# vmonardo/pnp-svrg

Hardware: AMD Instinct MI355X
Metric: PnP-SVRG inner-iters/sec, 256x256 CSMRI+DnCNN (higher is better)
Workload: dtype f32; 1 GPU; pnp_svrg (true SVRG direction, T2=10, mb=1000) on 256x256 CSMRI, 20% Bernoulli mask, DnCNN-17 prox (reference DnCNN_noise15 weights); batch_per_gpu=120, problems_total=120, parallelism=replicas x1 (no data-path collective)

## Files before the change

include/pnp_hip.h:

```cpp
#ifndef PNP_HIP_H
#define PNP_HIP_H
#include <stddef.h>
#include <stdint.h>

#ifdef __cplusplus
extern "C" {
#endif

enum { PNP_F32 = 0, PNP_F64 = 1 };
enum { PNP_OK = 0, PNP_ERR_ARG = 1, PNP_ERR_HIP = 2, PNP_ERR_UNSUPPORTED = 3 };

int pnp_version(void);
const char* pnp_last_error(void);

typedef struct pnp_csmri_plan pnp_csmri_plan;

int pnp_csmri_plan_create(pnp_csmri_plan** plan, int H, int W, int batch, int dtype);
int pnp_csmri_plan_destroy(pnp_csmri_plan* plan);

int pnp_csmri_sel_from_indices(pnp_csmri_plan* plan, const int32_t* idx, int n, uint8_t* selT, void* stream);
int pnp_csmri_pack_mask(pnp_csmri_plan* plan, const uint8_t* selT, uint32_t* bitsT, void* stream);

int pnp_csmri_draw_thresholds(pnp_csmri_plan* plan, const uint32_t* bitsT, int mb, uint64_t seed, uint32_t step0,
                              int nsteps, const uint32_t* step_dev, void* mbd, uint32_t* selbits, void* stream);
int pnp_csmri_sel_from_thresholds(pnp_csmri_plan* plan, const uint32_t* bitsT, const void* mbd, uint8_t* selT,
                                  void* stream);
int pnp_csmri_draw_minibatch(pnp_csmri_plan* plan, const uint32_t* bitsT, int mb, uint64_t seed, uint32_t step,
                             const uint32_t* step_dev, uint8_t* selT, void* stream);
int pnp_csmri_sel_from_dense(pnp_csmri_plan* plan, const uint8_t* sel, uint8_t* selT, void* stream);

int pnp_csmri_pack_y(pnp_csmri_plan* plan, const void* YT, const uint8_t* selT, void* yh, void* stream);

int pnp_csmri_grad(pnp_csmri_plan* plan, const void* a, const void* b, const uint8_t* selT,
                   const void* yh, double alpha, double beta, const void* c1,
                   double gamma, const void* c2, void* out, void* stream);

int pnp_csmri_grad_sel(pnp_csmri_plan* plan, const void* a, const void* b, const uint8_t* selT, const uint32_t* bitsT,
                       const void* yh, const void* YT, double alpha, const void* alpha_vec, double beta,
                       const void* c1, double gamma, const void* c2, void* out, void* stream);

int pnp_csmri_svrg_step(pnp_csmri_plan* plan, const void* a, const void* b, const uint32_t* bitsT, double alpha,
                        const void* alpha_vec, double beta, const void* c1, double gamma, const void* c2, void* out,
                        int denoise, double sigma_modifier, double fallback_sigma, const void* xrec, double* sse_out,
                        void* sigma_out, void* stream);

int pnp_csmri_svrg_outer_step(pnp_csmri_plan* plan, const void* z, const uint32_t* mask_bitsT, const void* yh,
                              const void* alpha_vec, double lr, void* w_out, void* mu_out, void* out, int denoise,
                              double sigma_modifier, double fallback_sigma, const void* xrec, double* sse_out,
                              void* sigma_out, void* stream);

int pnp_csmri_svrg_outer_iteration(pnp_csmri_plan* plan, void* z, void* w, void* mu, const uint32_t* mask_bitsT, const void* yh,
                                   const void* alpha_vec, const uint32_t* selbits, int T2, double lr, int mini_batch_size,
                                   double sigma_modifier, double fallback_sigma, const void* xrec, double* sse_log,
                                   int log_row0, int n_log, void* sigma_out, void* stream);

typedef struct pnp_deblur_plan pnp_deblur_plan;
int pnp_deblur_plan_create(pnp_deblur_plan** plan, int H, int W, int batch, int dtype, const void* Bk, int M,
                           const int32_t* g_idx, const void* g_w, const int32_t* a_rowptr,
                           const int32_t* a_col, const void* a_val);
int pnp_deblur_plan_destroy(pnp_deblur_plan* plan);
int pnp_deblur_grad(pnp_deblur_plan* plan, const void* z, const void* Y, const uint8_t* sel, double scale,
                    void* out, void* stream);
int pnp_deblur_grad_mb(pnp_deblur_plan* plan, const void* z, const void* Y, const void* mbd, double scale,
                       void* out, void* stream);
int pnp_deblur_forward(pnp_deblur_plan* plan, const void* x, void* out, void* stream);

size_t pnp_pr_workspace_elems(int M, int N);
int pnp_pr_grad(const void* A, const void* w, const void* y, const int32_t* rows, int nsel, int M, int N,
                int dtype, double scale, void* workspace, void* out, void* stream);
int pnp_pr_grad_batch(const void* A, const void* w, const void* y, const int32_t* rows, int nsel, int M, int N, int batch,
                      int dtype, double scale, void* workspace, void* out, void* stream);
int pnp_pr_spectral_apply(const void* A, const void* v, const void* y, int M, int N, int dtype, double scale,
                          void* workspace, void* out, void* stream);

int pnp_sigma_est(const void* z, int H, int W, int batch, int dtype, void* sigma_out, void* stream);

int pnp_prox_tv(const void* z_in, void* z_out, int H, int W, int batch, int dtype,
                const void* sigma_in, double sigma_modifier, double fallback_sigma,
                const void* xrec, double* sse_out, void* sigma_out, void* stream);

int pnp_nlm2d(const void* z_in, void* z_out, int H, int W, int batch, int dtype, int patch_size,
              int patch_distance, const void* sigma_in, double sigma_modifier, double fixed_h,
              const double* w0, double w0_sum, const void* xrec, double* sse_out, double* sse_workspace,
              void* stream);

int pnp_sse(const void* z, const void* xrec, int n_per_problem, int batch, int dtype, double* sse_out, void* stream);

int pnp_minmax(const void* z, int n_per_problem, int batch, int dtype, void* out, void* stream);

typedef struct pnp_dncnn_plan pnp_dncnn_plan;
int pnp_dncnn_plan_create(pnp_dncnn_plan** plan, int n_mid, const float* w_first, const float* w_mid,
                          const float* b_mid, const float* w_last, int H, int W, int batch);
int pnp_dncnn_plan_destroy(pnp_dncnn_plan* plan);
int pnp_dncnn_set_affine(pnp_dncnn_plan* plan, const float* b_first, float b_last, float negative_slope);
int pnp_dncnn_set_winograd(pnp_dncnn_plan* plan, int enable);
int pnp_dncnn_forward(pnp_dncnn_plan* plan, const float* x, float* r, void* stream);
int pnp_dncnn_denoise(pnp_dncnn_plan* plan, const void* z_in, void* z_out, int dtype, double sigma_net,
                      const void* xrec, double* sse_out, void* stream);

int pnp_mmo_denoise(pnp_dncnn_plan* plan, const void* z_in, void* z_out, int dtype, const void* xrec,
                    double* sse_out, void* stream);

int pnp_dncnn_profile_begin(pnp_dncnn_plan* plan, int max_calls);
int pnp_dncnn_profile_end(pnp_dncnn_plan* plan, double* avg_ms_per_launch, long* launches);
int pnp_dncnn_debug_clock(pnp_dncnn_plan* plan, int reps, double* cycles, double* ref_ticks, void* stream);
size_t pnp_dncnn_debug_w44_floats(void);
int pnp_dncnn_debug_w44_weights(pnp_dncnn_plan* plan, int layer, float* dst, void* stream);
int pnp_dncnn_debug_mid_layer(pnp_dncnn_plan* plan, int layer, const float* in, float* out, const float* w44_override,
                              int w44_rows, void* stream);
int pnp_dncnn_debug_fused_last(pnp_dncnn_plan* plan, const float* in, float* part, int w44_rows, void* stream);

int pnp_counter_add(uint32_t* counter, uint32_t inc, void* stream);
int pnp_log_append(const double* src, int n, double* log, int n_log, const uint32_t* step_dev, void* stream);
int pnp_log_append_inc(const double* src, int n, double* log, int n_log, uint32_t* counter, void* stream);

int pnp_draw_thresholds(int M, int batch, int mb, uint64_t seed, uint32_t step0, int nsteps, const uint32_t* step_dev,
                        void* mbd, void* stream);
int pnp_indicator_from_thresholds(int M, int batch, const void* mbd, uint8_t* sel, void* stream);
int pnp_rows_from_thresholds(int M, int batch, int mb, const void* mbd, int32_t* rows, void* stream);
int pnp_indicator_from_indices(const int32_t* idx, int n, int M, int batch, uint8_t* sel, void* stream);
int pnp_saga_table_update(void* z, const void* g, void* slot, const void* prev, void* sum, double lr, double inv_hist,
                          size_t n, int dtype, void* stream);

int pnp_axpbypcz(double a, const void* x, double b, const void* y, double c, const void* w,
                 void* out, size_t n, int dtype, void* stream);

int pnp_legacy_choice(uint32_t* mt_key, int* mt_pos, const int64_t* pool, int pop, int size, int32_t* work, int64_t* out);

#ifdef __cplusplus
}
#endif
#endif
```

pnp_svrg_amd/_native.py:

```python
import ctypes
import os

_HERE = os.path.dirname(os.path.abspath(__file__))
LIB_PATH = os.environ.get('PNP_HIP_LIB') or os.path.join(_HERE, 'lib', 'libpnp_hip.so')

F32, F64 = 0, 1

_vp = ctypes.c_void_p
_i = ctypes.c_int
_d = ctypes.c_double
_sz = ctypes.c_size_t

SIGNATURES = {
    'pnp_version': (_i, []),
    'pnp_last_error': (ctypes.c_char_p, []),
    'pnp_csmri_plan_create': (_i, [ctypes.POINTER(_vp), _i, _i, _i, _i]),
    'pnp_csmri_plan_destroy': (_i, [_vp]),
    'pnp_csmri_sel_from_indices': (_i, [_vp, _vp, _i, _vp, _vp]),
    'pnp_csmri_pack_mask': (_i, [_vp, _vp, _vp, _vp]),
    'pnp_csmri_draw_thresholds': (_i, [_vp, _vp, _i, ctypes.c_uint64, ctypes.c_uint32, _i, _vp, _vp, _vp, _vp]),
    'pnp_csmri_sel_from_thresholds': (_i, [_vp, _vp, _vp, _vp, _vp]),
    'pnp_csmri_draw_minibatch': (_i, [_vp, _vp, _i, ctypes.c_uint64, ctypes.c_uint32, _vp, _vp, _vp]),
    'pnp_counter_add': (_i, [_vp, ctypes.c_uint32, _vp]),
    'pnp_log_append': (_i, [_vp, _i, _vp, _i, _vp, _vp]),
    'pnp_log_append_inc': (_i, [_vp, _i, _vp, _i, _vp, _vp]),
    'pnp_csmri_sel_from_dense': (_i, [_vp, _vp, _vp, _vp]),
    'pnp_csmri_pack_y': (_i, [_vp, _vp, _vp, _vp, _vp]),
    'pnp_csmri_grad': (_i, [_vp, _vp, _vp, _vp, _vp, _d, _d, _vp, _d, _vp, _vp, _vp]),
    'pnp_csmri_grad_sel': (_i, [_vp, _vp, _vp, _vp, _vp, _vp, _vp, _d, _vp, _d, _vp, _d, _vp, _vp, _vp]),
    'pnp_csmri_svrg_step': (_i, [_vp, _vp, _vp, _vp, _d, _vp, _d, _vp, _d, _vp, _vp, _i, _d, _d, _vp, _vp, _vp, _vp]),
    'pnp_csmri_svrg_outer_step': (_i, [_vp, _vp, _vp, _vp, _vp, _d, _vp, _vp, _vp, _i, _d, _d, _vp, _vp, _vp, _vp]),
    'pnp_csmri_svrg_outer_iteration': (_i, [_vp, _vp, _vp, _vp, _vp, _vp, _vp, _vp, _i, _d, _i, _d, _d, _vp, _vp, _i, _i, _vp, _vp]),
    'pnp_deblur_plan_create': (_i, [ctypes.POINTER(_vp), _i, _i, _i, _i, _vp, _i, _vp, _vp, _vp, _vp, _vp]),
    'pnp_deblur_plan_destroy': (_i, [_vp]),
    'pnp_deblur_grad': (_i, [_vp, _vp, _vp, _vp, _d, _vp, _vp]),
    'pnp_deblur_grad_mb': (_i, [_vp, _vp, _vp, _vp, _d, _vp, _vp]),
    'pnp_deblur_forward': (_i, [_vp, _vp, _vp, _vp]),
    'pnp_pr_workspace_elems': (_sz, [_i, _i]),
    'pnp_pr_grad': (_i, [_vp, _vp, _vp, _vp, _i, _i, _i, _i, _d, _vp, _vp, _vp]),
    'pnp_pr_grad_batch': (_i, [_vp, _vp, _vp, _vp, _i, _i, _i, _i, _i, _d, _vp, _vp, _vp]),
    'pnp_pr_spectral_apply': (_i, [_vp, _vp, _vp, _i, _i, _i, _d, _vp, _vp, _vp]),
    'pnp_sigma_est': (_i, [_vp, _i, _i, _i, _i, _vp, _vp]),
    'pnp_prox_tv': (_i, [_vp, _vp, _i, _i, _i, _i, _vp, _d, _d, _vp, _vp, _vp, _vp]),
    'pnp_nlm2d': (_i, [_vp, _vp, _i, _i, _i, _i, _i, _i, _vp, _d, _d, _vp, _d, _vp, _vp, _vp, _vp]),
    'pnp_sse': (_i, [_vp, _vp, _i, _i, _i, _vp, _vp]),
    'pnp_minmax': (_i, [_vp, _i, _i, _i, _vp, _vp]),
    'pnp_dncnn_plan_create': (_i, [ctypes.POINTER(_vp), _i, _vp, _vp, _vp, _vp, _i, _i, _i]),
    'pnp_dncnn_plan_destroy': (_i, [_vp]),
    'pnp_dncnn_set_affine': (_i, [_vp, _vp, ctypes.c_float, ctypes.c_float]),
    'pnp_dncnn_set_winograd': (_i, [_vp, _i]),
    'pnp_dncnn_forward': (_i, [_vp, _vp, _vp, _vp]),
    'pnp_dncnn_denoise': (_i, [_vp, _vp, _vp, _i, _d, _vp, _vp, _vp]),
    'pnp_mmo_denoise': (_i, [_vp, _vp, _vp, _i, _vp, _vp, _vp]),
    'pnp_dncnn_profile_begin': (_i, [_vp, _i]),
    'pnp_dncnn_profile_end': (_i, [_vp, ctypes.POINTER(_d), ctypes.POINTER(ctypes.c_long)]),
    'pnp_dncnn_debug_clock': (_i, [_vp, _i, ctypes.POINTER(_d), ctypes.POINTER(_d), _vp]),
    'pnp_dncnn_debug_w44_floats': (_sz, []),
    'pnp_dncnn_debug_w44_weights': (_i, [_vp, _i, _vp, _vp]),
    'pnp_dncnn_debug_mid_layer': (_i, [_vp, _i, _vp, _vp, _vp, _i, _vp]),
    'pnp_dncnn_debug_fused_last': (_i, [_vp, _vp, _vp, _i, _vp]),
    'pnp_draw_thresholds': (_i, [_i, _i, _i, ctypes.c_uint64, ctypes.c_uint32, _i, _vp, _vp, _vp]),
    'pnp_indicator_from_thresholds': (_i, [_i, _i, _vp, _vp, _vp]),
    'pnp_rows_from_thresholds': (_i, [_i, _i, _i, _vp, _vp, _vp]),
    'pnp_indicator_from_indices': (_i, [_vp, _i, _i, _i, _vp, _vp]),
    'pnp_saga_table_update': (_i, [_vp, _vp, _vp, _vp, _vp, _d, _d, _sz, _i, _vp]),
    'pnp_axpbypcz': (_i, [_d, _vp, _d, _vp, _d, _vp, _vp, _sz, _i, _vp]),
    'pnp_legacy_choice': (_i, [_vp, ctypes.POINTER(ctypes.c_int), _vp, _i, _i, _vp, _vp]),
}

_lib = None


class NativeError(RuntimeError):
    pass


def lib():
    global _lib
    if _lib is None:
        if not os.path.exists(LIB_PATH):
            raise NativeError(
                f'{LIB_PATH} not found: build it with `python -c "import __graft_entry__ as g; g.build()"` '
                '(or `make -C pnp_svrg_amd/csrc`). There is no CPU fallback.')
        h = ctypes.CDLL(LIB_PATH)
        for name, (res, args) in SIGNATURES.items():
            fn = getattr(h, name)
            fn.restype = res
            fn.argtypes = args
        _lib = h
    return _lib


def check(status, what=''):
    if status != 0:
        msg = lib().pnp_last_error().decode(errors='replace')
        raise NativeError(f'{what} failed (status {status}): {msg}')


def call(name, *args):
    check(getattr(lib(), name)(*args), name)
```

pnp_svrg_amd/csrc/dncnn.hip:

```cpp
#include "direct.h"
#include "wino44.h"
#include "wino44b.h"
#include "reduce.h"
#include <vector>
#include <algorithm>
#include <cstdlib>
#include <type_traits>

namespace pnp {

constexpr int C = 64;

template <typename T>
__global__ __launch_bounds__(256) void k_first(const T* __restrict__ z, const T* __restrict__ mm,
                                               const float* __restrict__ w, const float* __restrict__ bfirst,
                                               float* __restrict__ out, int H, int W, double srange, double sshift,
                                               int clamp01, float slope) {
    __shared__ float ws[C * 9];
    __shared__ float bs[C];
    for (int i = threadIdx.x; i < C * 9; i += 256) ws[i] = w[i];
    if (threadIdx.x < C) bs[threadIdx.x] = bfirst[threadIdx.x];
    __syncthreads();
    const int b = blockIdx.y;
    const int p = blockIdx.x * 256 + threadIdx.x;
    if (p >= H * W) return;
    const int y = p / W, x = p - y * W;
    const T lo = mm ? mm[2 * b] : (T)0, hi = mm ? mm[2 * b + 1] : (T)1;
    const T* zi = z + (size_t)b * H * W;
    float v[9];
#pragma unroll
    for (int t = 0; t < 9; ++t) {
        const int yy = y + t / 3 - 1, xx = x + t % 3 - 1;
        float q = 0.f;
        if (yy >= 0 && yy < H && xx >= 0 && xx < W) {
            T u = zi[yy * W + xx];
            if (clamp01) {
                u = u < (T)0 ? (T)0 : (u > (T)1 ? (T)1 : u);
            } else {
                u = (u - lo) / (hi - lo);
                u = u * (T)srange + (T)sshift;
            }
            q = (float)u;
        }
        v[t] = q;
    }
#pragma unroll 4
    for (int c = 0; c < C; ++c) {
        float a = 0.f;
#pragma unroll
        for (int t = 0; t < 9; ++t) a = fmaf(ws[c * 9 + t], v[t], a);
        a += bs[c];
        out[((size_t)b * C + c) * H * W + p] = a > 0.f ? a : slope * a + 0.f;
    }
}

constexpr int LT_R = 16, LT_C = 64, LT_CK = 4, LT_PR = LT_R + 2, LT_PC = LT_C + 8;

template <typename T>
__global__ __launch_bounds__(256) void k_last(const float* __restrict__ act, const float* __restrict__ w,
                                              const T* zin, const T* __restrict__ mm,
                                              T* zout, float* __restrict__ r_out,
                                              const T* __restrict__ xrec, double* __restrict__ sse_part, int H, int W,
                                              double srange, double sshift, int skip01, float blast) {
    __shared__ float ws[C * 9];
    __shared__ __attribute__((aligned(16))) float tile[LT_CK * LT_PR * LT_PC];
    __shared__ double red[4];
    const int tid = threadIdx.x;
    for (int i = tid; i < C * 9; i += 256) ws[i] = w[i];
    const int b = blockIdx.z;
    const int ty0 = blockIdx.y * LT_R, tx0 = blockIdx.x * LT_C;
    const int py = tid >> 4, px = (tid & 15) * 4;
    const float* ab = act + (size_t)b * C * H * W;
    float r[4] = {0.f, 0.f, 0.f, 0.f};
    constexpr int SLAB = LT_CK * LT_PR * (LT_PC / 4);
    constexpr int PER_T = (SLAB + 255) / 256;
    float4 pre[PER_T];
    auto fetch = [&](int c0) {
#pragma unroll
        for (int k = 0; k < PER_T; ++k) {
            const int i = tid + 256 * k;
            float4 v = make_float4(0.f, 0.f, 0.f, 0.f);
            if (i < SLAB) {
                const int ch = i / (LT_PR * (LT_PC / 4)), rem = i - ch * (LT_PR * (LT_PC / 4));
                const int ry = rem / (LT_PC / 4), cx = rem - ry * (LT_PC / 4);
                const int y = ty0 - 1 + ry, x = tx0 - 4 + 4 * cx;
                if (y >= 0 && y < H && x >= 0 && x < W)
                    v = *reinterpret_cast<const float4*>(ab + ((size_t)(c0 + ch) * H + y) * W + x);
            }
            pre[k] = v;
        }
    };
    fetch(0);
    for (int c0 = 0; c0 < C; c0 += LT_CK) {
        __syncthreads();
#pragma unroll
        for (int k = 0; k < PER_T; ++k) {
            const int i = tid + 256 * k;
            if (i < SLAB) reinterpret_cast<float4*>(tile)[i] = pre[k];
        }
        __syncthreads();
        if (c0 + LT_CK < C) fetch(c0 + LT_CK);
#pragma unroll
        for (int ch = 0; ch < LT_CK; ++ch) {
            const float* wc = ws + (c0 + ch) * 9;
#pragma unroll
            for (int dy = 0; dy < 3; ++dy) {
                const float* row = tile + (ch * LT_PR + py + dy) * LT_PC + px + 4;
                const float4 m = *reinterpret_cast<const float4*>(row);
                const float l = row[-1], rr = row[4];
                const float w0 = wc[dy * 3], w1 = wc[dy * 3 + 1], w2 = wc[dy * 3 + 2];
                r[0] = fmaf(w0, l, fmaf(w1, m.x, fmaf(w2, m.y, r[0])));
                r[1] = fmaf(w0, m.x, fmaf(w1, m.y, fmaf(w2, m.z, r[1])));
                r[2] = fmaf(w0, m.y, fmaf(w1, m.z, fmaf(w2, m.w, r[2])));
                r[3] = fmaf(w0, m.z, fmaf(w1, m.w, fmaf(w2, rr, r[3])));
            }
        }
    }
    double err = 0.0;
    const int y = ty0 + py;
    if (y < H) {
#pragma unroll
        for (int j = 0; j < 4; ++j) {
            const int x = tx0 + px + j;
            if (x >= W) continue;
            const size_t p = (size_t)b * H * W + (size_t)y * W + x;
            r[j] += blast;
            if (r_out != nullptr) r_out[p] = r[j];
            if (zout != nullptr && skip01) {
                const float xin = (float)zin[p];
                float v = (xin < 0.f ? 0.f : (xin > 1.f ? 1.f : xin)) + r[j];
                v = v < 0.f ? 0.f : (v > 1.f ? 1.f : v);
                zout[p] = (T)v;
                if (xrec != nullptr) {
                    const double d = (double)xrec[p] - (double)(T)v;
                    err += d * d;
                }
            } else if (zout != nullptr) {
                const T lo = mm[2 * b], hi = mm[2 * b + 1];
                T v = (zin[p] - lo) / (hi - lo);
                v = v * (T)srange + (T)sshift;
                v = v - (T)r[j];
                v = (v - (T)sshift) / (T)srange;
                v = v * (hi - lo) + lo;
                zout[p] = v;
                if (xrec != nullptr) {
                    const double d = (double)xrec[p] - (double)v;
                    err += d * d;
                }
            }
        }
    }
    if (sse_part != nullptr) {
        err = wave_sum(err);
        if ((tid & 63) == 0) red[tid >> 6] = err;
        __syncthreads();
        if (tid == 0)
            sse_part[((size_t)b * gridDim.y + blockIdx.y) * gridDim.x + blockIdx.x] = red[0] + red[1] + red[2] + red[3];
    }
}

template <typename T>
__global__ __launch_bounds__(256) void k_last_patches(const float* __restrict__ part, const T* zin, const T* __restrict__ mm,
                                                      T* zout, float* __restrict__ r_out, const T* __restrict__ xrec,
                                                      double* __restrict__ sse_part, int H, int W, double srange, double sshift,
                                                      float blast) {
    __shared__ double red[4];
    const int tid = threadIdx.x, b = blockIdx.z;
    const int iy = tid >> 6, ix = tid & 3, bx = blockIdx.x * 16 + ((tid >> 2) & 15), by = blockIdx.y;
    const int y = 4 * by + iy, x = 4 * bx + ix;
    const int NBX = W / 4, NBY = H / 4;
    const float* pb = part + (size_t)b * NBY * NBX * 36;
    auto at = [&](int qy, int qx, int py, int px) { return pb[((size_t)qy * NBX + qx) * 36 + py * 6 + px]; };
    const int vy = iy == 0 ? -1 : iy == 3 ? 1 : 0, vx = ix == 0 ? -1 : ix == 3 ? 1 : 0;
    const bool hv = vy != 0 && by + vy >= 0 && by + vy < NBY, hh = vx != 0 && bx + vx >= 0 && bx + vx < NBX;
    const int py = iy + 1, px = ix + 1, pyn = py - 4 * vy, pxn = px - 4 * vx;
    float r = at(by, bx, py, px);
    if (hv) r += at(by + vy, bx, pyn, px);
    if (hh) r += at(by, bx + vx, py, pxn);
    if (hv && hh) r += at(by + vy, bx + vx, pyn, pxn);
    r += blast;
    const size_t p = (size_t)b * H * W + (size_t)y * W + x;
    if (r_out != nullptr) r_out[p] = r;
    double err = 0.0;
    if (zout != nullptr) {
        const T lo = mm ? mm[2 * b] : (T)0, hi = mm ? mm[2 * b + 1] : (T)1;
        T v = (zin[p] - lo) / (hi - lo);
        v = v * (T)srange + (T)sshift;
        v = v - (T)r;
        v = (v - (T)sshift) / (T)srange;
        v = v * (hi - lo) + lo;
        zout[p] = v;
        if (xrec != nullptr) {
            const double d = (double)xrec[p] - (double)v;
            err = d * d;
        }
    }
    if (sse_part != nullptr) {
        err = wave_sum(err);
        if ((tid & 63) == 0) red[tid >> 6] = err;
        __syncthreads();
        if (tid == 0)
            sse_part[((size_t)b * gridDim.y + blockIdx.y) * gridDim.x + blockIdx.x] = red[0] + red[1] + red[2] + red[3];
    }
}

__global__ void k_sum_parts(const double* __restrict__ part, int nparts, double* __restrict__ out) {
    double s = 0;
    for (int i = threadIdx.x; i < nparts; i += 64) s += part[(size_t)blockIdx.x * nparts + i];
    s = wave_sum(s);
    if (threadIdx.x == 0) out[blockIdx.x] = s;
}

}
using namespace pnp;

static const ConvMode kModes[] = {
    {0, direct_supports, direct_layer_bytes, direct_pack, direct_layer, direct_debug_clock, false},
    {1, direct_supports, wino23_layer_bytes, wino23_pack, wino23_layer, wino23_debug_clock, false},
    {5, wino44_supports, wino44_layer_bytes, wino44_pack, wino44_layer, wino44_debug_clock, true},
    {6, wino44b_supports, wino44b_layer_bytes, wino44b_pack, wino44b_layer, wino44b_debug_clock, false},
};
constexpr int NMODES = sizeof(kModes) / sizeof(kModes[0]);

static const ConvMode* find_mode(int mode) {
    for (const ConvMode& m : kModes)
        if (m.mode == mode) return &m;
    return nullptr;
}

static int resolve_conv_mode(int requested, int H, int W, bool strict, const ConvMode** out) {
    const ConvMode* m = find_mode(requested);
    PNP_CHECK_ARG(m || !strict,
                  "mode must be 0 (direct), 1 (Winograd F(2,3) along x), 5 (Winograd F(4x4,3x3)) or 6 (the same on 3 x bf16 splits)");
    if (!m) m = find_mode(5);
    PNP_CHECK_ARG(m->supports(H, W) || !strict, "Winograd F(4x4,3x3) needs H % 8 == 0 and W % 64 == 0");
    *out = m->supports(H, W) ? m : find_mode(1);
    return PNP_OK;
}

struct pnp_dncnn_plan {
    int n_mid, H, W, batch, num_cu;
    float *w_first, *w_last, *bias;
    void* wconv[NMODES];
    const ConvMode* conv;
    float* b_first;
    float b_last, slope;
    bool edge_fusion;
    float* part;
    float *act0, *act1, *zeros;
    double* mm;
    double* sse_part;
    bool profile;
    std::vector<hipEvent_t> ev;
    size_t ev_used;
    double prof_ms;
    long prof_launches;
};

static void plan_free(pnp_dncnn_plan* p) {
    for (void* q : p->wconv) (void)hipFree(q);
    for (void* q : {(void*)p->bias, (void*)p->w_first, (void*)p->w_last, (void*)p->act0, (void*)p->act1, (void*)p->zeros,
                    (void*)p->mm, (void*)p->sse_part, (void*)p->b_first, (void*)p->part})
        (void)hipFree(q);
    for (hipEvent_t e : p->ev) (void)hipEventDestroy(e);
    delete p;
}

static ConvLayerArgs conv_args(const pnp_dncnn_plan* p, int l, const float* in, float* out, hipStream_t s) {
    return {in, out, p->wconv[p->conv - kModes], l, p->bias + (size_t)l * C, p->zeros, p->H, p->W, p->batch, p->num_cu, p->slope, s};
}

extern "C" int pnp_dncnn_plan_create(pnp_dncnn_plan** out, int n_mid, const float* w_first, const float* w_mid,
                                     const float* b_mid, const float* w_last, int H, int W, int batch) {
    PNP_CHECK_ARG(out && w_first && w_mid && b_mid && w_last, "null argument");
    PNP_CHECK_ARG(n_mid >= 1 && batch >= 1, "n_mid and batch must be >= 1");
    PNP_CHECK_ARG(H % 8 == 0 && W % 32 == 0 && (H * W) % 256 == 0, "H must be a multiple of 8, W of 32");
    auto* p = new pnp_dncnn_plan{};
    p->n_mid = n_mid; p->H = H; p->W = W; p->batch = batch;
    hipDeviceProp_t prop;
    int dev = 0;
    PNP_CHECK_HIP(hipGetDevice(&dev));
    PNP_CHECK_HIP(hipGetDeviceProperties(&prop, dev));
    p->num_cu = prop.multiProcessorCount;
    const char* ev = getenv("PNP_DNCNN_WINOGRAD");
    (void)resolve_conv_mode(ev ? atoi(ev) : 5, H, W, false, &p->conv);
    const char* ef = getenv("PNP_DNCNN_EDGE_FUSION");
    p->edge_fusion = !(ef && atoi(ef) == 0);
    const size_t act_bytes = (size_t)batch * C * H * W * sizeof(float);
    hipError_t e = hipSuccess;
    auto alloc = [&](auto** dst, size_t bytes, const void* src = nullptr) {
        if (e == hipSuccess) e = hipMalloc(dst, bytes);
        if (e == hipSuccess && src) e = hipMemcpy(*dst, src, bytes, hipMemcpyHostToDevice);
    };
    for (int i = 0; i < NMODES; ++i) {
        if (!kModes[i].supports(H, W)) continue;
        std::vector<char> w(kModes[i].layer_bytes() * n_mid);
        kModes[i].pack(w_mid, n_mid, w.data());
        alloc(&p->wconv[i], w.size(), w.data());
    }
    alloc(&p->bias, (size_t)n_mid * C * sizeof(float), b_mid);
    alloc(&p->w_first, C * 9 * sizeof(float), w_first);
    alloc(&p->w_last, C * 9 * sizeof(float), w_last);
    alloc(&p->b_first, C * sizeof(float));
    if (e == hipSuccess) e = hipMemset(p->b_first, 0, C * sizeof(float));
    alloc(&p->act0, act_bytes);
    alloc(&p->act1, act_bytes);
    alloc(&p->zeros, 256);
    if (e == hipSuccess) e = hipMemset(p->zeros, 0, 256);
    alloc(&p->mm, (size_t)batch * 2 * sizeof(double));
    alloc(&p->sse_part, (size_t)batch * (H * W / 256) * sizeof(double));
    if (wino44_supports(H, W)) alloc(&p->part, wino44_part_floats(H, W, batch) * sizeof(float));
    if (e != hipSuccess) {
        set_error(std::string("pnp_dncnn_plan_create: ") + hipGetErrorString(e));
        plan_free(p);
        return PNP_ERR_HIP;
    }
    *out = p;
    return PNP_OK;
}

extern "C" int pnp_dncnn_plan_destroy(pnp_dncnn_plan* p) {
    if (p) plan_free(p);
    return PNP_OK;
}

namespace {
template <typename T>
int run_dncnn(pnp_dncnn_plan* p, const T* z_in, bool normalise, double sigma_net, T* z_out, float* r_out,
              const T* xrec, double* sse_out, hipStream_t s, bool mmo = false) {
    const int H = p->H, W = p->W, B = p->batch, HW = H * W;
    T* mm = normalise ? (T*)p->mm : nullptr;
    double srange = 1.0, sshift = 0.0;
    if (normalise) {
        k_minmax<T><<<B, 256, 0, s>>>(z_in, HW, mm);
        PNP_CHECK_LAUNCH();
        srange = 1.0 + sigma_net / 255.0 / 2.0;
        sshift = (1.0 - srange) / 2.0;
    }
    dim3 pg(HW / 256, B);
    k_first<T><<<pg, 256, 0, s>>>(z_in, mm, p->w_first, p->b_first, p->act0, H, W, srange, sshift, mmo ? 1 : 0, p->slope);
    PNP_CHECK_LAUNCH();
    float *src = p->act0, *dst = p->act1;
    const bool fuse_last = p->edge_fusion && p->conv->fuses_last && p->slope == 0.f && !mmo && std::is_same<T, float>::value &&
                           p->part != nullptr;
    const bool prof = p->profile && p->ev_used + 2 <= p->ev.size();
    if (prof) PNP_CHECK_HIP(hipEventRecord(p->ev[p->ev_used], s));
    for (int l = 0; l < p->n_mid; ++l) {
        ConvLayerArgs a = conv_args(p, l, src, dst, s);
        if (fuse_last && l == p->n_mid - 1) { a.wlast = p->w_last; a.part = p->part; }
        const int rc = p->conv->layer(a);
        if (rc != PNP_OK) return rc;
        std::swap(src, dst);
    }
    if (prof) { PNP_CHECK_HIP(hipEventRecord(p->ev[p->ev_used + 1], s)); p->ev_used += 2; }
    if (fuse_last) {
        const dim3 fg(W / 64, H / 4, B);
        k_last_patches<T><<<fg, 256, 0, s>>>(p->part, z_in, mm, z_out, r_out, xrec, sse_out ? p->sse_part : nullptr, H, W, srange,
                                             sshift, p->b_last);
        PNP_CHECK_LAUNCH();
        if (sse_out) {
            k_sum_parts<<<B, 64, 0, s>>>(p->sse_part, (int)(fg.x * fg.y), sse_out);
            PNP_CHECK_LAUNCH();
        }
        return PNP_OK;
    }
    dim3 lg((W + LT_C - 1) / LT_C, (H + LT_R - 1) / LT_R, B);
    k_last<T><<<lg, 256, 0, s>>>(src, p->w_last, z_in, mm, z_out, r_out, xrec, sse_out ? p->sse_part : nullptr, H, W,
                                 srange, sshift, mmo ? 1 : 0, p->b_last);
    PNP_CHECK_LAUNCH();
    if (sse_out) {
        k_sum_parts<<<B, 64, 0, s>>>(p->sse_part, (int)(lg.x * lg.y), sse_out);
        PNP_CHECK_LAUNCH();
    }
    return PNP_OK;
}
}

extern "C" size_t pnp_dncnn_debug_w44_floats(void) { return wino44_layer_bytes() / sizeof(float); }

extern "C" int pnp_dncnn_debug_w44_weights(pnp_dncnn_plan* p, int layer, float* dst, void* stream) {
    PNP_CHECK_ARG(p && dst && layer >= 0 && layer < p->n_mid, "bad argument");
    const char* w = (const char*)p->wconv[find_mode(5) - kModes];
    PNP_CHECK_ARG(w != nullptr, "the plan's image size rules out the F(4x4,3x3) kernel (mode 5): no such weights");
    PNP_CHECK_HIP(hipMemcpyAsync(dst, w + (size_t)layer * wino44_layer_bytes(), wino44_layer_bytes(), hipMemcpyDeviceToDevice,
                                 (hipStream_t)stream));
    return PNP_OK;
}

extern "C" int pnp_dncnn_debug_mid_layer(pnp_dncnn_plan* p, int layer, const float* in, float* out, const float* w44_override,
                                         int w44_rows, void* stream) {
    PNP_CHECK_ARG(p && in && out && layer >= 0 && layer < p->n_mid && w44_rows >= 0 && w44_rows <= 2, "bad argument");
    ConvLayerArgs a = conv_args(p, layer, in, out, (hipStream_t)stream);
    a.force_rows = w44_rows;
    a.w44_override = w44_override;
    return p->conv->layer(a);
}

extern "C" int pnp_dncnn_debug_fused_last(pnp_dncnn_plan* p, const float* in, float* part, int w44_rows, void* stream) {
    PNP_CHECK_ARG(p && in && part && w44_rows >= 0 && w44_rows <= 2, "bad argument");
    ConvLayerArgs a = conv_args(p, p->n_mid - 1, in, nullptr, (hipStream_t)stream);
    a.force_rows = w44_rows;
    a.wlast = p->w_last;
    a.part = part;
    return p->conv->layer(a);
}

extern "C" int pnp_dncnn_set_affine(pnp_dncnn_plan* p, const float* b_first, float b_last, float negative_slope) {
    PNP_CHECK_ARG(p != nullptr, "null plan");
    PNP_CHECK_ARG(negative_slope >= 0.f && negative_slope < 1.f, "negative_slope must be in [0, 1)");
    if (b_first) PNP_CHECK_HIP(hipMemcpy(p->b_first, b_first, C * sizeof(float), hipMemcpyHostToDevice));
    else PNP_CHECK_HIP(hipMemset(p->b_first, 0, C * sizeof(float)));
    p->b_last = b_last;
    p->slope = negative_slope;
    return PNP_OK;
}

extern "C" int pnp_dncnn_set_winograd(pnp_dncnn_plan* p, int enable) {
    PNP_CHECK_ARG(p != nullptr, "null plan");
    return resolve_conv_mode(enable, p->H, p->W, true, &p->conv);
}

extern "C" int pnp_dncnn_profile_begin(pnp_dncnn_plan* p, int max_calls) {
    PNP_CHECK_ARG(p && max_calls > 0, "bad argument");
    while (p->ev.size() < (size_t)2 * max_calls) {
        hipEvent_t e;
        PNP_CHECK_HIP(hipEventCreate(&e));
        p->ev.push_back(e);
    }
    p->profile = true; p->ev_used = 0; p->prof_ms = 0; p->prof_launches = 0;
    return PNP_OK;
}

extern "C" int pnp_dncnn_profile_end(pnp_dncnn_plan* p, double* avg_ms_per_launch, long* launches) {
    PNP_CHECK_ARG(p && avg_ms_per_launch && launches, "null argument");
    p->profile = false;
    for (size_t i = 0; i + 1 < p->ev_used; i += 2) {
        PNP_CHECK_HIP(hipEventSynchronize(p->ev[i + 1]));
        float ms = 0;
        PNP_CHECK_HIP(hipEventElapsedTime(&ms, p->ev[i], p->ev[i + 1]));
        p->prof_ms += ms;
        p->prof_launches += p->n_mid;
    }
    *launches = p->prof_launches;
    *avg_ms_per_launch = p->prof_launches ? p->prof_ms / (double)p->prof_launches : 0.0;
    return PNP_OK;
}

extern "C" int pnp_dncnn_debug_clock(pnp_dncnn_plan* p, int reps, double* cycles, double* ref_ticks, void* stream) {
    PNP_CHECK_ARG(p && cycles && ref_ticks && reps >= 1, "bad argument");
    std::vector<double> c, r;
    const int rc = p->conv->debug_clock(conv_args(p, 0, p->act0, p->act1, (hipStream_t)stream), reps, c, r);
    if (rc != PNP_OK) return rc;
    std::sort(c.begin(), c.end());
    std::sort(r.begin(), r.end());
    *cycles = c[c.size() / 2];
    *ref_ticks = r[r.size() / 2];
    return PNP_OK;
}

extern "C" int pnp_dncnn_forward(pnp_dncnn_plan* p, const float* x, float* r, void* stream) {
    PNP_CHECK_ARG(p && x && r, "null argument");
    return run_dncnn<float>(p, x, false, 0.0, nullptr, r, nullptr, nullptr, (hipStream_t)stream);
}

extern "C" int pnp_mmo_denoise(pnp_dncnn_plan* p, const void* z_in, void* z_out, int dtype, const void* xrec,
                               double* sse_out, void* stream) {
    PNP_CHECK_ARG(p && z_in && z_out, "null argument");
    PNP_CHECK_ARG(!(sse_out && !xrec), "sse_out needs xrec");
    if (dtype == PNP_F32)
        return run_dncnn<float>(p, (const float*)z_in, false, 0.0, (float*)z_out, nullptr, (const float*)xrec, sse_out,
                                (hipStream_t)stream, true);
    if (dtype == PNP_F64)
        return run_dncnn<double>(p, (const double*)z_in, false, 0.0, (double*)z_out, nullptr, (const double*)xrec, sse_out,
                                 (hipStream_t)stream, true);
    PNP_CHECK_ARG(false, "bad dtype");
}

extern "C" int pnp_dncnn_denoise(pnp_dncnn_plan* p, const void* z_in, void* z_out, int dtype, double sigma_net,
                                 const void* xrec, double* sse_out, void* stream) {
    PNP_CHECK_ARG(p && z_in && z_out, "null argument");
    PNP_CHECK_ARG(!(sse_out && !xrec), "sse_out needs xrec");
    if (dtype == PNP_F32)
        return run_dncnn<float>(p, (const float*)z_in, true, sigma_net, (float*)z_out, nullptr, (const float*)xrec, sse_out,
                                (hipStream_t)stream);
    if (dtype == PNP_F64)
        return run_dncnn<double>(p, (const double*)z_in, true, sigma_net, (double*)z_out, nullptr, (const double*)xrec,
                                 sse_out, (hipStream_t)stream);
    PNP_CHECK_ARG(false, "bad dtype");
}
```

pnp_svrg_amd/csrc/dncnn_conv.h:

```cpp
#pragma once
#include "common.h"
#include <vector>

namespace pnp {

struct ConvLayerArgs {
    const float* in;
    float* out;
    const void* w;
    int layer;
    const float *bias, *zeros;
    int H, W, batch, num_cu;
    float slope;
    hipStream_t s;
    int force_rows = 0;
    const float* w44_override = nullptr;
    const float* wlast = nullptr;
    float* part = nullptr;
};

struct ConvMode {
    int mode;
    bool (*supports)(int H, int W);
    size_t (*layer_bytes)();
    void (*pack)(const float* w_mid, int n_mid, void* out);
    int (*layer)(const ConvLayerArgs& a);
    int (*debug_clock)(const ConvLayerArgs& a, int reps, std::vector<double>& cycles, std::vector<double>& ticks);
    bool fuses_last;
};

inline int check_plain_conv(const ConvLayerArgs& a) {
    PNP_CHECK_ARG(a.w44_override == nullptr, "w44_override needs the F(4x4,3x3) kernel (mode 5)");
    PNP_CHECK_ARG(a.part == nullptr, "the fused last layer needs the F(4x4,3x3) kernel (mode 5) and ReLU");
    return PNP_OK;
}

template <typename F>
int read_stamps(hipStream_t s, int nwg, int per_wg, F&& launch, std::vector<unsigned long long>& h, std::vector<double>& cycles,
                std::vector<double>& ticks) {
    unsigned long long* d = nullptr;
    PNP_CHECK_HIP(hipMalloc(&d, (size_t)nwg * per_wg * sizeof(*d)));
    h.resize((size_t)nwg * per_wg);
    const int rc = launch(d);
    hipError_t e = rc != PNP_OK ? hipSuccess : hipMemcpyAsync(h.data(), d, h.size() * sizeof(*d), hipMemcpyDeviceToHost, s);
    if (rc == PNP_OK && e == hipSuccess) e = hipStreamSynchronize(s);
    (void)hipFree(d);
    if (rc != PNP_OK) return rc;
    PNP_CHECK_HIP(e);
    for (int i = 0; i < nwg; ++i) { cycles.push_back((double)h[(size_t)per_wg * i]); ticks.push_back((double)h[(size_t)per_wg * i + 1]); }
    return PNP_OK;
}

}
```

pnp_svrg_amd/csrc/dncnn_wino44.hip:

```cpp
#include "common.h"
#include "wino44.h"
#include "tilewalk.h"
#include <vector>
#include <utility>
#include <cstdlib>

namespace pnp {
namespace w44 {

using f32x4 = __attribute__((ext_vector_type(4))) float;
using f32x2 = __attribute__((ext_vector_type(2))) float;

constexpr int C = 64;
constexpr int TC = 64;
constexpr int PC = 72;
constexpr int KC = 8;
constexpr int NCH = C / KC;
template <int NG_> struct Geo {
    static constexpr int NG = NG_;
    static constexpr int TR = 4 * NG, PR = TR + 2;
    static constexpr int PLANE = NG == 2 ? 768 : 512;
    static constexpr int DBUF = KC * PLANE;
    static constexpr int PPW = DBUF / 256 / 4;
    static constexpr int VPL = 128 * NG;
    static constexpr int VBUF = 36 * VPL;
    static constexpr int LDS_FLOATS = 2 * DBUF + 2 * VBUF;
    static constexpr int NQ_AGPR = NG == 2 ? 64 : 36;
    static constexpr bool in_agpr(int g, int xi) { return g * 36 + xi < NQ_AGPR; }
};
constexpr int URING = 18;
constexpr unsigned DUMMY = 1u << 27;

__device__ __forceinline__ void bt6(float d0, float d1, float d2, float d3, float d4, float d5, float (&v)[6]) {
    const float t1 = __builtin_fmaf(-4.f, d2, d4), t2 = __builtin_fmaf(-4.f, d1, d3);
    const float t3 = d4 - d2, sd = d3 - d1;
    v[0] = __builtin_fmaf(4.f, d0, __builtin_fmaf(-5.f, d2, d4));
    v[1] = t1 + t2;
    v[2] = t1 - t2;
    v[3] = __builtin_fmaf(2.f, sd, t3);
    v[4] = __builtin_fmaf(-2.f, sd, t3);
    v[5] = __builtin_fmaf(4.f, d1, __builtin_fmaf(-5.f, d3, d5));
}
template <typename T> __device__ __forceinline__ void at6(T m0, T m1, T m2, T m3, T m4, T m5, T (&y)[4]) {
    const T s12 = m1 + m2, d12 = m1 - m2, s34 = m3 + m4, d34 = m3 - m4;
    y[0] = (m0 + s12) + s34;
    y[1] = 2.f * d34 + d12;
    y[2] = 4.f * s34 + s12;
    y[3] = (8.f * d34 + d12) + m5;
}

#define PNP_MFMA_PRE ""
#define PNP_MFMA_POST ""
template <bool AG> __device__ __forceinline__ void mfma(f32x4& acc, float w, float v) {
    if (AG) asm volatile(PNP_MFMA_PRE "v_mfma_f32_16x16x4_f32 %0, %1, %2, %0" PNP_MFMA_POST : "+a"(acc) : "v"(w), "v"(v));
    else asm volatile(PNP_MFMA_PRE "v_mfma_f32_16x16x4_f32 %0, %1, %2, %0" PNP_MFMA_POST : "+v"(acc) : "v"(w), "v"(v));
}
template <bool AG> __device__ __forceinline__ void mfma_first(f32x4& acc, float w, float v) {
    if (AG) asm volatile("v_mfma_f32_16x16x4_f32 %0, %1, %2, 0" PNP_MFMA_POST : "=&a"(acc) : "v"(w), "v"(v));
    else asm volatile("v_mfma_f32_16x16x4_f32 %0, %1, %2, 0" PNP_MFMA_POST : "=&v"(acc) : "v"(w), "v"(v));
}

typedef int i32x4 __attribute__((ext_vector_type(4)));
typedef __attribute__((address_space(3))) float lds_f;
typedef __attribute__((address_space(3))) f32x2 lds_f2;
typedef __attribute__((address_space(3))) f32x4 lds_f4;

__device__ __forceinline__ void dma_piece_asm(unsigned voff, i32x4 rsrc, unsigned lds_byte_addr) {
    asm volatile("s_mov_b32 m0, %2\n\ts_nop 0\n\tbuffer_load_dwordx4 %0, %1, 0 offen lds" :: "v"(voff), "s"(rsrc), "s"(lds_byte_addr) : "memory");
}

struct Patch {
    f32x2 a; f32x4 m; f32x2 e;
    f32x2 t[6][3];
    f32x2 v[6];
};
template <int NG_> struct Ctx {
    static constexpr int NG = NG_;
    using G = Geo<NG_>;
    f32x4 acc[NG_][36];
    f32x4 ur[URING];
    Patch P;
    f32x2 b[2][NG_];
    const lds_f* dsrc[2];
    lds_f* vdst[2];
    const lds_f* vsrc0[2];
    const lds_f* vsrc1[2];
    const __attribute__((address_space(1))) char* ucur;
    unsigned ulane;
    __device__ __forceinline__ f32x4 uload_next() {
        const f32x4 u = *(const __attribute__((address_space(1))) f32x4*)(ucur + ulane);
        ucur += 1024;
        asm volatile("" : "+s"(ucur));
        return u;
    }
};
#define PNP_SLOT() __builtin_amdgcn_sched_barrier(0)

template <int DPAR, int R, int HALF, typename CT> __device__ __forceinline__ void patch_load(CT& c) {
    const lds_f* row = c.dsrc[DPAR] + R * PC;
    if (HALF == 0) { c.P.a = *(const lds_f2*)(row + 2); c.P.e = *(const lds_f2*)(row + 8); }
    else c.P.m = *(const lds_f4*)(row + 4);
}
__device__ __forceinline__ f32x2 pk_sum_diff(f32x2 a) {
    f32x2 r;
    asm("v_pk_add_f32 %0, %1, %1 op_sel:[0,1] op_sel_hi:[1,0] neg_hi:[0,1]" : "=v"(r) : "v"(a));
    return r;
}
__device__ __forceinline__ f32x2 pk_hi_pm_2lo(f32x2 a) {
    f32x2 r;
    asm("v_pk_fma_f32 %0, %1, 2.0, %1 op_sel:[0,0,1] op_sel_hi:[0,0,1] neg_hi:[1,0,0]" : "=v"(r) : "v"(a));
    return r;
}
__device__ __forceinline__ void bt6_pk(f32x2 q0, f32x2 q1, f32x2 q2, f32x2 q3, f32x2 q4, f32x2 q5, f32x2 (&v)[6]) {
    const f32x2 t1 = q4 - 4.f * q2, t2 = q3 - 4.f * q1;
    const f32x2 t3 = q4 - q2, sd = q3 - q1;
    v[0] = 4.f * q0 + (q4 - 5.f * q2);
    v[1] = t1 + t2;
    v[2] = t1 - t2;
    v[3] = 2.f * sd + t3;
    v[4] = t3 - 2.f * sd;
    v[5] = 4.f * q1 + (q5 - 5.f * q3);
}
constexpr int col_pair(int sl) { return (sl - 6) / 2; }
constexpr bool is_col_slice(int sl) { return sl == 6 || sl == 8 || sl == 10; }
template <int SL, typename CT> __device__ __forceinline__ void slice_valu(CT& c) {
    Patch& P = c.P;
    if constexpr (SL < 6) {
        asm volatile("" :: "v"(P.a.x), "v"(P.e.y));
        const f32x2 p12 = {P.m.x, P.m.y}, p34 = {P.m.z, P.m.w};
        const f32x2 A = p34 - 4.f * p12;
        const f32x2 Bv = p34 - p12;
        P.t[SL][1] = pk_sum_diff(A);
        P.t[SL][2] = pk_hi_pm_2lo(Bv);
        float v0, v5;
        asm("v_fma_f32 %0, 4.0, %1, %2" : "=v"(v0) : "v"(P.a.y), "v"(__builtin_fmaf(-5.f, P.m.y, P.m.w)));
        asm("v_fma_f32 %0, 4.0, %1, %2" : "=v"(v5) : "v"(P.m.x), "v"(__builtin_fmaf(-5.f, P.m.z, P.e.x)));
        P.t[SL][0] = f32x2{v0, v5};
    } else if constexpr (is_col_slice(SL)) {
        constexpr int cp = col_pair(SL);
        bt6_pk(P.t[0][cp], P.t[1][cp], P.t[2][cp], P.t[3][cp], P.t[4][cp], P.t[5][cp], P.v);
    }
}
template <int DPAR, int SL, int N, typename CT> __device__ __forceinline__ void slice_lds(CT& c) {
    constexpr int VPL = CT::G::VPL;
    if constexpr (SL < 5) {
        if constexpr (N < 2) patch_load<DPAR, SL + 1, N>(c);
    } else if constexpr (is_col_slice(SL)) {
        constexpr int cp = col_pair(SL), xa = cp == 0 ? 0 : cp == 1 ? 1 : 3, xb = cp == 0 ? 5 : cp == 1 ? 2 : 4;
#pragma unroll
        for (int y = 2 * N; y < 2 * N + 2; ++y) {
            c.vdst[DPAR][(y * 6 + xa) * VPL] = c.P.v[y].x;
            c.vdst[DPAR][(y * 6 + xb) * VPL] = c.P.v[y].y;
        }
    }
}
template <int VPAR, int XI, int GR, typename CT> __device__ __forceinline__ void b_load(CT& c) {
    if constexpr (GR < CT::NG) {
        if (GR == 0) c.b[XI & 1][0] = *(const lds_f2*)(c.vsrc0[VPAR] + XI * CT::G::VPL);
        else c.b[XI & 1][GR] = *(const lds_f2*)(c.vsrc1[VPAR] + XI * CT::G::VPL);
    }
}
template <int K, int XI, int GR, typename CT> __device__ __forceinline__ void mfma_j0(CT& c, float u, f32x2 (&b)[CT::NG]) {
    if constexpr (GR < CT::NG) {
        if constexpr (K == 0) mfma_first<CT::G::in_agpr(GR, XI)>(c.acc[GR][XI], u, b[GR].x);
        else mfma<CT::G::in_agpr(GR, XI)>(c.acc[GR][XI], u, b[GR].x);
    }
}
template <int XI, int GR, typename CT> __device__ __forceinline__ void mfma_j1(CT& c, float u, f32x2 (&b)[CT::NG]) {
    if constexpr (GR < CT::NG) mfma<CT::G::in_agpr(GR, XI)>(c.acc[GR][XI], u, b[GR].y);
}

template <int K, int P, int VAR, typename CT, typename DMA> __device__ __forceinline__ void step(CT& c, DMA&& dma) {
    constexpr int X0 = 2 * P, X1 = 2 * P + 1, SQ = K * 18 + P;
    constexpr int VPAR = K & 1, DPAR = (K + 1) & 1, NG = CT::NG;
    const f32x4 u = c.ur[SQ % URING];
    f32x2 b0[NG], b1[NG];
#pragma unroll
    for (int g = 0; g < NG; ++g) b0[g] = c.b[0][g];
    mfma_j0<K, X0, 0>(c, u.x, b0);                   PNP_SLOT();
    if constexpr (VAR != 13 && VAR != 15) b_load<VPAR, X1, 0>(c);
    PNP_SLOT();
    mfma_j0<K, X0, 1>(c, u.x, b0);                   PNP_SLOT();
    if constexpr (VAR != 13 && VAR != 15) b_load<VPAR, X1, 1>(c);
    PNP_SLOT();
    mfma_j1<X0, 0>(c, u.y, b0);                      PNP_SLOT();
    if constexpr (VAR != 10 && VAR != 15) slice_valu<P>(c);
    PNP_SLOT();
    mfma_j1<X0, 1>(c, u.y, b0);                      PNP_SLOT();
    if constexpr (VAR != 14 && VAR != 15) slice_lds<DPAR, P, 0>(c);
    PNP_SLOT();
#pragma unroll
    for (int g = 0; g < NG; ++g) b1[g] = c.b[1][g];
    mfma_j0<K, X1, 0>(c, u.z, b1);                   PNP_SLOT();
    if constexpr (X1 + 1 < 36 && VAR != 13 && VAR != 15) b_load<VPAR, X1 + 1, 0>(c);
    PNP_SLOT();
    mfma_j0<K, X1, 1>(c, u.z, b1);                   PNP_SLOT();
    if constexpr (X1 + 1 < 36 && VAR != 13 && VAR != 15) b_load<VPAR, X1 + 1, 1>(c);
    PNP_SLOT();
    mfma_j1<X1, 0>(c, u.w, b1);                      PNP_SLOT();
    if constexpr (P < CT::G::PPW && VAR != 11 && VAR != 15) dma(P);
    if constexpr (VAR != 14 && VAR != 15) slice_lds<DPAR, P, 1>(c);
    PNP_SLOT();
    mfma_j1<X1, 1>(c, u.w, b1);                      PNP_SLOT();
    if constexpr (VAR != 14 && VAR != 15) slice_lds<DPAR, P, 2>(c);
    if constexpr (VAR != 12 && VAR != 15 && SQ + URING < NCH * 18) c.ur[SQ % URING] = c.uload_next();
    PNP_SLOT();
}
template <int K, int VAR, typename CT, typename DMA, int... P> __device__ __forceinline__ void chunk_steps(CT& c, DMA&& dma, std::integer_sequence<int, P...>) {
    (step<K, P, VAR>(c, dma), ...);
}
template <int K> constexpr int reloads_from(int p0) {
    int n = 0;
    for (int p = p0; p < 18; ++p) n += (K * 18 + p + URING < NCH * 18) ? 1 : 0;
    return n;
}
template <int K, bool STAMP, int VAR, typename CT, typename DMA> __device__ __forceinline__ void chunk(CT& c, DMA&& dma, unsigned long long& t_wait) {
    patch_load<(K + 1) & 1, 0, 0>(c);
    patch_load<(K + 1) & 1, 0, 1>(c);
    b_load<K & 1, 0, 0>(c);
    b_load<K & 1, 0, 1>(c);
    PNP_SLOT();
    chunk_steps<K, VAR>(c, dma, std::make_integer_sequence<int, 18>{});
    unsigned long long ta = 0;
    if (STAMP) ta = __builtin_amdgcn_s_memtime();
    asm volatile("s_waitcnt vmcnt(%0)" :: "n"(reloads_from<K>(CT::G::PPW)) : "memory");
    __syncthreads();
    if (STAMP) t_wait += __builtin_amdgcn_s_memtime() - ta;
}
template <bool STAMP, int VAR, typename CT, typename MK, int... K> __device__ __forceinline__ void all_chunks(CT& c, MK&& mk, unsigned long long& t_wait, std::integer_sequence<int, K...>) {
    (chunk<K, STAMP, VAR>(c, mk(std::integral_constant<int, K>{}), t_wait), ...);
}

template <int VPL> __device__ __forceinline__ void transform0(const float* dsrc, float* vdst) {
    float t[6][6];
#pragma unroll
    for (int r = 0; r < 6; ++r) {
        const float* row = dsrc + r * PC;
        bt6(row[3], row[4], row[5], row[6], row[7], row[8], t[r]);
    }
#pragma unroll
    for (int x = 0; x < 6; ++x) {
        float v[6];
        bt6(t[0][x], t[1][x], t[2][x], t[3][x], t[4][x], t[5][x], v);
#pragma unroll
        for (int y = 0; y < 6; ++y) vdst[(y * 6 + x) * VPL] = v[y];
    }
}

constexpr int FL_PATCH = 36;
constexpr int FL_BLK = 16 * FL_PATCH;
template <int NG, bool FL> constexpr int fl_lds_floats() { return FL ? C * 9 + NG * 4 * FL_BLK : 0; }

template <bool LEAKY, int NG = 2, bool STAMP = false, int VAR = 0, bool FL = false>
__global__ __launch_bounds__(256, 1) void k_mid_wino44(const float* __restrict__ in, float* __restrict__ out,
                                                       const float4* __restrict__ upack, const float* __restrict__ bias,
                                                       int H, int W, int ntiles, float slope,
                                                       unsigned long long* __restrict__ stamps = nullptr, int tile0 = 0,
                                                       const float* __restrict__ wlast = nullptr, float* __restrict__ part = nullptr) {
    using G = Geo<NG>;
    constexpr int TR = G::TR, PR = G::PR, PLANE = G::PLANE, DBUF = G::DBUF, PPW = G::PPW, VPL = G::VPL, VBUF = G::VBUF;
    static_assert(!(FL && LEAKY), "the fused last layer is built for the ReLU net");
    __shared__ __attribute__((aligned(16))) float lds[G::LDS_FLOATS + fl_lds_floats<NG, FL>()];
    const int tid = threadIdx.x, lane = tid & 63, wv = __builtin_amdgcn_readfirstlane(tid >> 6);
    const int tiles_x = W / TC, units_per_img = tiles_x * (H / 8);
    auto region = [&](int u, int& b, int& ty0, int& tx0) {
        const int t = tile0 + (NG == 2 ? u : u >> 1);
        b = t / units_per_img;
        const int t2 = t - b * units_per_img;
        ty0 = (t2 / tiles_x) * 8 + (NG == 2 ? 0 : 4 * (u & 1));
        tx0 = (t2 % tiles_x) * TC;
    };

    float bv[4];
#pragma unroll
    for (int r = 0; r < 4; ++r) bv[r] = bias[16 * wv + 4 * (lane >> 4) + r];

    const int tc = lane & 15, j = (lane >> 4) & 1, g = NG == 2 ? lane >> 5 : 0;
    const int d_off = 4 * ((2 * wv + j) * (PLANE / 4) + g * PC + tc);
    const ptrdiff_t hw4 = (ptrdiff_t)4 * H * W, w4 = (ptrdiff_t)4 * W;
    const unsigned st_off = 4u * (unsigned)(4 * (lane >> 4) * H * W + 4 * tc);
    const int v_off = g * 128 + wv * 32 + tc * 2 + j;

    unsigned pdesc[PPW];
#pragma unroll
    for (int i = 0; i < PPW; ++i) {
        const int q = (wv + 4 * i) * 64 + lane;
        const int c = q / (PLANE / 4), r = q - c * (PLANE / 4);
        const int ry = r / 18, cx4 = 4 * (r - ry * 18);
        const unsigned edge = (ry == 0 ? 1u : 0u) | (ry == PR - 1 ? 2u : 0u) | (cx4 == 0 ? 4u : 0u) | (cx4 == TC + 4 ? 8u : 0u);
        pdesc[i] = r < PR * 18 ? ((unsigned)((c * H + ry) * W + cx4) | (edge << 28)) : DUMMY;
    }
    const unsigned lds0 = (unsigned)(size_t)(__attribute__((address_space(3))) float*)lds;
    struct TileDma { size_t base; unsigned voff[PPW]; };
    const size_t chunk_bytes = (size_t)KC * H * W * 4;
    auto tile_dma = [&](int t) {
        TileDma td;
        int b, ty0, tx0;
        region(t, b, ty0, tx0);
        td.base = (size_t)in + 4 * ((((size_t)b * C) * H + ty0 - 1) * (size_t)W + tx0 - 4);
        const unsigned bad = t < ntiles ? ((((ty0 == 0 ? 1u : 0u) | (ty0 + TR == H ? 2u : 0u) | (tx0 == 0 ? 4u : 0u) | (tx0 + TC == W ? 8u : 0u)) << 28) | DUMMY)
                                        : 0xFFFFFFFFu;
#pragma unroll
        for (int i = 0; i < PPW; ++i) td.voff[i] = (pdesc[i] & bad) == 0u ? 4u * (pdesc[i] & 0x07FFFFFFu) : 0x80000000u;
        return td;
    };
    auto chunk_rsrc = [&](const TileDma& td, int k) {
        const size_t base = td.base + (size_t)k * chunk_bytes;
        i32x4 rs;
        rs.x = (int)(unsigned)base; rs.y = (int)(unsigned)(base >> 32) & 0xFFFF; rs.z = (int)0x80000000u; rs.w = 0x00020000;
        return rs;
    };
    auto dma_piece = [&](const TileDma& td, i32x4 rs, int buf, int i) {
        dma_piece_asm(td.voff[i], rs, lds0 + 4u * (unsigned)(buf * DBUF + (wv + 4 * i) * 256));
    };

    float* const dbuf = lds;
    float* const vbuf = lds + 2 * DBUF;

    Ctx<NG> c;
    lds_f* const ldsp = (lds_f*)lds;
    c.dsrc[0] = ldsp + d_off;                     c.dsrc[1] = ldsp + DBUF + d_off;
    c.vdst[0] = ldsp + 2 * DBUF + v_off;          c.vdst[1] = ldsp + 2 * DBUF + VBUF + v_off;
    c.vsrc0[0] = ldsp + 2 * DBUF + 2 * lane;      c.vsrc0[1] = ldsp + 2 * DBUF + VBUF + 2 * lane;
    c.vsrc1[0] = c.vsrc0[0] + 128;                c.vsrc1[1] = c.vsrc0[1] + 128;
    asm volatile("" : "+v"(c.vsrc1[0]), "+v"(c.vsrc1[1]));
    const __attribute__((address_space(1))) char* const ubase = (const __attribute__((address_space(1))) char*)upack + (size_t)(wv * NCH * 18) * 1024;
    c.ucur = ubase;
    c.ulane = 16u * lane;

    const TileWalk tw_ = tile_walk(ntiles);
    int tile = tw_.first;
    const int limit = tw_.limit < ntiles ? tw_.limit : ntiles;
    float* const flw = lds + G::LDS_FLOATS;
    float* const flx = flw + C * 9;
    if constexpr (FL)
        for (int i = tid; i < C * 9; i += 256) flw[i] = wlast[i];
    {
        const TileDma td0 = tile_dma(tile < limit ? tile : ntiles);
#pragma unroll
        for (int i = 0; i < PPW; ++i) dma_piece(td0, chunk_rsrc(td0, 0), 0, i);
#pragma unroll
        for (int i = 0; i < PPW; ++i) dma_piece(td0, chunk_rsrc(td0, 1), 1, i);
#pragma unroll
        for (int i = 0; i < URING; ++i) c.ur[i] = c.uload_next();
        asm volatile("s_waitcnt vmcnt(0)" ::: "memory");
        __syncthreads();
        transform0<VPL>(dbuf + d_off, vbuf + v_off);
        __syncthreads();
    }

    unsigned long long t0 = 0, r0 = 0, t_wait = 0, t_epi = 0;
    if (STAMP) { t0 = __builtin_amdgcn_s_memtime(); r0 = __builtin_amdgcn_s_memrealtime(); }
    for (; tile < limit; tile += tw_.step) {
        asm volatile("" : "+v"(c.ulane));
        int b, ty0, tx0;
        region(tile, b, ty0, tx0);
        const int ntile = tile + tw_.step < limit ? tile + tw_.step : ntiles;

        const TileDma cur = tile_dma(tile), nxt = tile_dma(ntile);
        all_chunks<STAMP, VAR>(c, [&](auto kc) {
            constexpr int K = decltype(kc)::value;
            const TileDma& td = K + 2 < NCH ? cur : nxt;
            const i32x4 rs = chunk_rsrc(td, (K + 2) % NCH);
            return [&, rs](int piece) { dma_piece(td, rs, K & 1, piece); };
        }, t_wait, std::make_integer_sequence<int, NCH>{});

        unsigned long long te = 0;
        if (STAMP) te = __builtin_amdgcn_s_memtime();
        asm volatile("; W44_EPILOGUE_BEGIN\n\ts_nop 15\n\ts_nop 7" ::: "memory");
#pragma unroll
        for (int g2 = 0; g2 < NG; ++g2)
#pragma unroll
            for (int xi = 0; xi < 36; xi += 4) {
                if (G::in_agpr(g2, xi)) asm volatile("" : "+a"(c.acc[g2][xi]), "+a"(c.acc[g2][xi + 1]), "+a"(c.acc[g2][xi + 2]), "+a"(c.acc[g2][xi + 3]));
                else asm volatile("" : "+v"(c.acc[g2][xi]), "+v"(c.acc[g2][xi + 1]), "+v"(c.acc[g2][xi + 2]), "+v"(c.acc[g2][xi + 3]));
            }
        unsigned so = st_off;
        asm volatile("" : "+v"(so));
        __attribute__((address_space(1))) char* const ob = (__attribute__((address_space(1))) char*)out + 4 * ((((size_t)b * C + 16 * wv) * H + ty0) * (size_t)W + tx0);
        float q[FL_PATCH];
#pragma unroll
        for (int blk = 0; blk < 2 * NG; ++blk) {
            {
                const int g2 = NG == 2 ? 1 - (blk >> 1) : 0, pi = blk & 1;
                float wr[2][9];
                if constexpr (FL) {
                    if (pi == 0)
#pragma unroll
                        for (int i = 0; i < FL_PATCH; ++i) q[i] = 0.f;
                    const float* wc = flw + (16 * wv + 4 * (lane >> 4) + 2 * pi) * 9;
#pragma unroll
                    for (int t = 0; t < 9; ++t) { wr[0][t] = wc[t]; wr[1][t] = wc[9 + t]; }
                }
                if (blk == 2 * NG - 1) {
                    c.ucur = ubase;
#pragma unroll
                    for (int i = 0; i < URING; ++i) c.ur[i] = c.uload_next();
                    __builtin_amdgcn_sched_barrier(0);
                }
                const f32x2 bias2 = {bv[2 * pi], bv[2 * pi + 1]};
                __attribute__((address_space(1))) char* oc = ob + (ptrdiff_t)(2 * pi) * hw4 + (ptrdiff_t)(4 * g2) * w4;
                asm volatile("" : "+s"(oc));
                f32x2 s[6][4];
#pragma unroll
                for (int x = 0; x < 6; ++x) {
                    f32x2 m[6];
#pragma unroll
                    for (int y = 0; y < 6; ++y) {
                        const f32x4 q = c.acc[g2][6 * y + x];
                        m[y] = pi ? f32x2{q.z, q.w} : f32x2{q.x, q.y};
                    }
                    if (x == 1) m[1] += bias2;
                    at6(m[0], m[1], m[2], m[3], m[4], m[5], s[x]);
                    if (x & 1) __builtin_amdgcn_sched_barrier(0);
                }
#pragma unroll
                for (int r = 0; r < 4; ++r) {
                    f32x2 y[4];
                    at6(s[0][r], s[1][r], s[2][r], s[3][r], s[4][r], s[5][r], y);
                    f32x4 v0, v1;
                    if (LEAKY) {
                        v0.x = fmaxf(y[0].x, slope * y[0].x); v0.y = fmaxf(y[1].x, slope * y[1].x);
                        v0.z = fmaxf(y[2].x, slope * y[2].x); v0.w = fmaxf(y[3].x, slope * y[3].x);
                        v1.x = fmaxf(y[0].y, slope * y[0].y); v1.y = fmaxf(y[1].y, slope * y[1].y);
                        v1.z = fmaxf(y[2].y, slope * y[2].y); v1.w = fmaxf(y[3].y, slope * y[3].y);
                    } else {
                        v0.x = fmaxf(y[0].x, 0.f); v0.y = fmaxf(y[1].x, 0.f); v0.z = fmaxf(y[2].x, 0.f); v0.w = fmaxf(y[3].x, 0.f);
                        v1.x = fmaxf(y[0].y, 0.f); v1.y = fmaxf(y[1].y, 0.f); v1.z = fmaxf(y[2].y, 0.f); v1.w = fmaxf(y[3].y, 0.f);
                    }
                    if constexpr (FL) {
                        const float a0[4] = {v0.x, v0.y, v0.z, v0.w}, a1[4] = {v1.x, v1.y, v1.z, v1.w};
#pragma unroll
                        for (int dy = 0; dy < 3; ++dy)
#pragma unroll
                            for (int dx = 0; dx < 3; ++dx)
#pragma unroll
                                for (int k = 0; k < 4; ++k) {
                                    float& d = q[(r + 2 - dy) * 6 + k + 2 - dx];
                                    d = __builtin_fmaf(wr[0][dy * 3 + dx], a0[k], d);
                                    d = __builtin_fmaf(wr[1][dy * 3 + dx], a1[k], d);
                                }
                    } else {
                        *(__attribute__((address_space(1))) f32x4*)(oc + so) = v0;
                        oc += hw4;
                        asm volatile("" : "+s"(oc));
                        *(__attribute__((address_space(1))) f32x4*)(oc + so) = v1;
                        oc += w4 - hw4;
                        asm volatile("" : "+s"(oc));
                    }
                    if (r & 1) __builtin_amdgcn_sched_barrier(0);
                }
                if constexpr (FL) {
                    if (pi == 1) {
                        const bool h32 = (lane & 32) != 0, h16 = (lane & 16) != 0;
                        float k1[18], k2[9];
#pragma unroll
                        for (int i = 0; i < 18; ++i) {
                            const float mine = h32 ? q[18 + i] : q[i], give = h32 ? q[i] : q[18 + i];
                            k1[i] = mine + __shfl_xor(give, 32);
                        }
#pragma unroll
                        for (int i = 0; i < 9; ++i) {
                            const float mine = h16 ? k1[9 + i] : k1[i], give = h16 ? k1[i] : k1[9 + i];
                            k2[i] = mine + __shfl_xor(give, 16);
                        }
                        float* const xd = flx + (g2 * 4 + wv) * FL_BLK + tc * FL_PATCH + 9 * (lane >> 4);
#pragma unroll
                        for (int i = 0; i < 9; ++i) xd[i] = k2[i];
                    }
                }
            }
        }
        if constexpr (FL) {
            __syncthreads();
            float* const pb = part + (((size_t)b * (H / 4) + ty0 / 4) * (size_t)(W / 4) + tx0 / 4) * FL_PATCH;
            for (int e = tid; e < NG * FL_BLK; e += 256) {
                const int g2 = e >= FL_BLK ? 1 : 0, rem = e - g2 * FL_BLK;
                const float* xs = flx + g2 * 4 * FL_BLK + rem;
                pb[(size_t)g2 * (W / 4) * FL_PATCH + rem] = ((xs[0] + xs[FL_BLK]) + xs[2 * FL_BLK]) + xs[3 * FL_BLK];
            }
        }
        asm volatile("; W44_EPILOGUE_END" ::: "memory");
        if (STAMP) t_epi += __builtin_amdgcn_s_memtime() - te;
    }
    if (STAMP && tid == 0) {
        stamps[4 * blockIdx.x] = __builtin_amdgcn_s_memtime() - t0;
        stamps[4 * blockIdx.x + 1] = __builtin_amdgcn_s_memrealtime() - r0;
        stamps[4 * blockIdx.x + 2] = t_wait;
        stamps[4 * blockIdx.x + 3] = t_epi;
    }
}

}

bool wino44_supports(int H, int W) { return H % 8 == 0 && W % w44::TC == 0; }

size_t wino44_layer_bytes() { return (size_t)4 * w44::NCH * 18 * 64 * 4 * sizeof(float); }

void wino44_pack(const float* w_mid, int n_mid, void* out_) {
    static const double G[6][3] = {{1.0 / 4, 0, 0}, {-1.0 / 6, -1.0 / 6, -1.0 / 6}, {-1.0 / 6, 1.0 / 6, -1.0 / 6},
                                   {1.0 / 24, 1.0 / 12, 1.0 / 6}, {1.0 / 24, -1.0 / 12, 1.0 / 6}, {0, 0, 1}};
    float* out = (float*)out_;
    for (int l = 0; l < n_mid; ++l)
        for (int wv = 0; wv < 4; ++wv)
            for (int k = 0; k < w44::NCH; ++k)
                for (int lane = 0; lane < 64; ++lane)
                    for (int j = 0; j < 2; ++j) {
                        const int cout = 16 * wv + (lane & 15), cin = w44::KC * k + 2 * (lane >> 4) + j;
                        const float* g = w_mid + (((size_t)l * w44::C + cout) * w44::C + cin) * 9;
                        for (int xy = 0; xy < 6; ++xy)
                            for (int xx = 0; xx < 6; ++xx) {
                                double u = 0;
                                for (int dy = 0; dy < 3; ++dy)
                                    for (int dx = 0; dx < 3; ++dx) u += G[xy][dy] * G[xx][dx] * (double)g[dy * 3 + dx];
                                const int xi = 6 * xy + xx, p = xi >> 1, e = 2 * (xi & 1) + j;
                                out[((((size_t)(l * 4 + wv) * w44::NCH + k) * 18 + p) * 64 + lane) * 4 + e] = (float)u;
                            }
                    }
}

int wino44_layer(const ConvLayerArgs& a) {
    PNP_CHECK_ARG(a.part == nullptr || (a.slope == 0.f && a.wlast != nullptr), "the fused last layer needs ReLU and w_last");
    const float *in = a.in, *bias = a.bias, *wlast = a.wlast;
    float *out = a.out, *part = a.part;
    const int H = a.H, W = a.W, num_cu = a.num_cu, force = a.force_rows, batch = a.batch;
    const float slope = a.slope;
    const hipStream_t s = a.s;
    const int units = batch * (H / 8) * (W / w44::TC);
    int full = force == 1 ? 0 : force == 2 ? units : (units / num_cu) * num_cu;
    if (force == 0 && 2 * (units - full) > num_cu) full = units;
    const float4* up = (const float4*)(a.w44_override ? a.w44_override : (const float*)a.w + a.layer * wino44_layer_bytes() / sizeof(float));
    if (full > 0) {
        const int grid = full < num_cu ? full : num_cu;
        if (part) w44::k_mid_wino44<false, 2, false, 0, true><<<grid, 256, 0, s>>>(in, out, up, bias, H, W, full, 0.f, nullptr, 0, wlast, part);
        else if (slope != 0.f) w44::k_mid_wino44<true, 2><<<grid, 256, 0, s>>>(in, out, up, bias, H, W, full, slope, nullptr, 0);
        else w44::k_mid_wino44<false, 2><<<grid, 256, 0, s>>>(in, out, up, bias, H, W, full, 0.f, nullptr, 0);
        PNP_CHECK_LAUNCH();
    }
    if (full < units) {
        const int n1 = 2 * (units - full), grid = n1 < num_cu ? n1 : num_cu;
        if (part) w44::k_mid_wino44<false, 1, false, 0, true><<<grid, 256, 0, s>>>(in, out, up, bias, H, W, n1, 0.f, nullptr, full, wlast, part);
        else if (slope != 0.f) w44::k_mid_wino44<true, 1><<<grid, 256, 0, s>>>(in, out, up, bias, H, W, n1, slope, nullptr, full);
        else w44::k_mid_wino44<false, 1><<<grid, 256, 0, s>>>(in, out, up, bias, H, W, n1, 0.f, nullptr, full);
        PNP_CHECK_LAUNCH();
    }
    return PNP_OK;
}

int wino44_debug_clock(const ConvLayerArgs& a, int reps, std::vector<double>& cycles, std::vector<double>& ticks) {
    const int ntiles = a.batch * (a.H / 8) * (a.W / w44::TC);
    const int grid = ntiles < a.num_cu ? ntiles : a.num_cu;
    const float *in = a.in, *bias = a.bias;
    float* out = a.out;
    const int H = a.H, W = a.W;
    const hipStream_t s = a.s;
    const float* upack_layer = (const float*)a.w + a.layer * wino44_layer_bytes() / sizeof(float);
    std::vector<unsigned long long> h;
    const int rc = read_stamps(s, grid, 4, [&](unsigned long long* stamps_dev) {
        for (int i = 0; i < reps - 1; ++i)
            w44::k_mid_wino44<false, 2><<<grid, 256, 0, s>>>(in, out, (const float4*)upack_layer, bias, H, W, ntiles, 0.f);
        const int var = getenv("PNP_W44_VAR") ? atoi(getenv("PNP_W44_VAR")) : 0;
        if (var == 0) w44::k_mid_wino44<false, 2, true><<<grid, 256, 0, s>>>(in, out, (const float4*)upack_layer, bias, H, W, ntiles, 0.f, stamps_dev);
#ifdef PNP_W44_ABLATIONS
#define PNP_W44_ABL(V) else if (var == V) w44::k_mid_wino44<false, 2, true, V><<<grid, 256, 0, s>>>(in, out, (const float4*)upack_layer, bias, H, W, ntiles, 0.f, stamps_dev);
        PNP_W44_ABL(10) PNP_W44_ABL(11) PNP_W44_ABL(12) PNP_W44_ABL(13) PNP_W44_ABL(14) PNP_W44_ABL(15)
#undef PNP_W44_ABL
#endif
        else PNP_CHECK_ARG(false, "PNP_W44_VAR: this library was built without -DPNP_W44_ABLATIONS");
        PNP_CHECK_LAUNCH();
        return PNP_OK;
    }, h, cycles, ticks);
    if (rc != PNP_OK) return rc;
    if (getenv("PNP_DEBUG_STAMPS")) {
        double wsum = 0, esum = 0, rsum = 0;
        for (int i = 0; i < grid; ++i) { wsum += (double)(h[4 * i + 2] & 0xFFFFFFFFull); rsum += (double)(h[4 * i + 2] >> 32); esum += h[4 * i + 3]; }
        fprintf(stderr, "[k_mid_wino44 stamps] mean cycles per WG: chunk-end wait + barrier %.0f  epilogue %.0f  (mode 6: steps 0..5 of the chunks %.0f)\n",
                wsum / grid, esum / grid, rsum / grid);
    }
    return PNP_OK;
}

}
```

pnp_svrg_amd/csrc/wino44.h:

```cpp
#pragma once
#include "dncnn_conv.h"

namespace pnp {
bool wino44_supports(int H, int W);
size_t wino44_layer_bytes();
void wino44_pack(const float* w_mid, int n_mid, void* out);
int wino44_layer(const ConvLayerArgs& a);
inline size_t wino44_part_floats(int H, int W, int batch) { return (size_t)batch * (H / 4) * (W / 4) * 36; }
int wino44_debug_clock(const ConvLayerArgs& a, int reps, std::vector<double>& cycles, std::vector<double>& ticks);
}
```

pnp_svrg_amd/ops.py:

```python
import ctypes
import torch
from . import _native as N

_DT = {torch.float32: N.F32, torch.float64: N.F64}
_CDT = {torch.float32: torch.complex64, torch.float64: torch.complex128}


def _stream():
    try:
        return ctypes.c_void_p(torch._C._cuda_getCurrentRawStream(torch._C._cuda_getDevice()))
    except AttributeError:
        return ctypes.c_void_p(torch.cuda.current_stream().cuda_stream)


def _p(t):
    if t is None:
        return None
    assert t.is_cuda and t.is_contiguous(), 'device-resident contiguous tensors only'
    return ctypes.c_void_p(t.data_ptr())


def require_gpu():
    if not torch.cuda.is_available():
        raise N.NativeError('no MI355X visible (torch.cuda.is_available() is False); the hot path has no CPU fallback')
    N.lib()


class CsmriPlan:

    def __init__(self, H, W, batch, dtype=torch.float32):
        require_gpu()
        self.H, self.W, self.B, self.dtype = H, W, batch, dtype
        h = ctypes.c_void_p()
        N.call('pnp_csmri_plan_create', ctypes.byref(h), H, W, batch, _DT[dtype])
        self._h = h

    def __del__(self):
        h, self._h = getattr(self, '_h', None), None
        if h:
            try:
                N.lib().pnp_csmri_plan_destroy(h)
            except Exception:
                pass

    def sel_from_indices(self, idx, out=None):
        assert idx.dtype == torch.int32 and idx.shape[0] == self.B
        out = out if out is not None else torch.empty((self.B, self.W, self.H), dtype=torch.uint8, device=idx.device)
        N.call('pnp_csmri_sel_from_indices', self._h, _p(idx), idx.shape[1], _p(out), _stream())
        return out

    def pack_mask(self, selT, out=None):
        assert selT.dtype == torch.uint8 and tuple(selT.shape) == (self.B, self.W, self.H)
        out = out if out is not None else torch.empty((self.B, self.W, self.H // 32), dtype=torch.int32, device=selT.device)
        N.call('pnp_csmri_pack_mask', self._h, _p(selT), _p(out), _stream())
        return out

    def draw_thresholds(self, bits, mb, seed, step0, nsteps=1, out=None, step_dev=None, selbits=None):
        assert bits.dtype == torch.int32 and tuple(bits.shape) == (self.B, self.W, self.H // 32)
        out = out if out is not None else torch.empty((nsteps, self.B, 2), dtype=torch.int64, device=bits.device)
        assert out.dtype == torch.int64 and tuple(out.shape) == (nsteps, self.B, 2)
        assert selbits is None or (selbits.dtype == torch.int32 and tuple(selbits.shape) == (nsteps, self.B, self.W, self.H // 32))
        N.call('pnp_csmri_draw_thresholds', self._h, _p(bits), int(mb), int(seed) & (2 ** 64 - 1), int(step0) & 0xFFFFFFFF,
               int(nsteps), _p(step_dev), _p(out), _p(selbits), _stream())
        return out

    def sel_from_thresholds(self, bits, mbd, out=None):
        assert mbd.dtype == torch.int64 and tuple(mbd.shape) == (self.B, 2)
        out = out if out is not None else torch.empty((self.B, self.W, self.H), dtype=torch.uint8, device=bits.device)
        N.call('pnp_csmri_sel_from_thresholds', self._h, _p(bits), _p(mbd), _p(out), _stream())
        return out

    def draw_minibatch(self, bits, mb, seed, step, out=None, step_dev=None):
        assert bits.dtype == torch.int32 and tuple(bits.shape) == (self.B, self.W, self.H // 32)
        out = out if out is not None else torch.empty((self.B, self.W, self.H), dtype=torch.uint8, device=bits.device)
        N.call('pnp_csmri_draw_minibatch', self._h, _p(bits), int(mb), int(seed) & (2 ** 64 - 1), int(step) & 0xFFFFFFFF,
               _p(step_dev), _p(out), _stream())
        return out

    def sel_from_dense(self, sel, out=None):
        assert sel.dtype == torch.uint8 and tuple(sel.shape) == (self.B, self.H, self.W)
        out = out if out is not None else torch.empty((self.B, self.W, self.H), dtype=torch.uint8, device=sel.device)
        N.call('pnp_csmri_sel_from_dense', self._h, _p(sel), _p(out), _stream())
        return out

    def pack_y(self, YT, selT, out=None):
        assert YT.dtype == _CDT[self.dtype] and tuple(YT.shape) == (self.B, self.W, self.H)
        out = out if out is not None else torch.empty((self.B, self.W // 2, self.H), dtype=YT.dtype, device=YT.device)
        N.call('pnp_csmri_pack_y', self._h, _p(YT), _p(selT), _p(out), _stream())
        return out

    def grad(self, a, selT=None, b=None, yh=None, alpha=1.0, beta=0.0, c1=None, gamma=0.0, c2=None, out=None, *,
             bits=None, alpha_vec=None, YT=None):
        for t in (a, b, c1, c2, out):
            assert t is None or (t.dtype == self.dtype and t.numel() == self.B * self.H * self.W)
        assert (selT is None) != (bits is None), 'pass selT or bits'
        assert alpha_vec is None or (alpha_vec.dtype == self.dtype and alpha_vec.numel() == self.B)
        out = out if out is not None else torch.empty_like(a)
        assert YT is None or (YT.dtype == _CDT[self.dtype] and tuple(YT.shape) == (self.B, self.W, self.H))
        N.call('pnp_csmri_grad_sel', self._h, _p(a), _p(b), _p(selT), _p(bits), _p(yh), _p(YT), float(alpha), _p(alpha_vec),
               float(beta), _p(c1), float(gamma), _p(c2), _p(out), _stream())
        return out


    def svrg_step(self, a, b, bits, alpha=1.0, beta=0.0, c1=None, gamma=0.0, c2=None, out=None, *, alpha_vec=None, denoise=True,
                  sigma_modifier=1.0, fallback_sigma=0.0, xrec=None, sse=None, sigma_out=None):
        assert self.dtype == torch.float32 and self.H == 256 and self.W == 256
        assert bits.dtype == torch.int32 and tuple(bits.shape) == (self.B, self.W, self.H // 32)
        out = out if out is not None else torch.empty_like(a)
        sigma_out = sigma_out if sigma_out is not None else torch.empty(self.B, dtype=a.dtype, device=a.device)
        N.call('pnp_csmri_svrg_step', self._h, _p(a), _p(b), _p(bits), float(alpha), _p(alpha_vec), float(beta), _p(c1),
               float(gamma), _p(c2), _p(out), 1 if denoise else 0, float(sigma_modifier), float(fallback_sigma), _p(xrec),
               _p(sse), _p(sigma_out), _stream())
        return out, sse, sigma_out


    def svrg_outer_step(self, z, mask_bits, yh, alpha_vec, lr, w_out, mu_out, out=None, *, denoise=True, sigma_modifier=1.0,
                        fallback_sigma=0.0, xrec=None, sse=None, sigma_out=None):
        assert self.dtype == torch.float32 and self.H == 256 and self.W == 256
        assert mask_bits.dtype == torch.int32 and tuple(mask_bits.shape) == (self.B, self.W, self.H // 32)
        for t in (z, w_out, mu_out, out):
            assert t is None or (t.dtype == self.dtype and t.numel() == self.B * self.H * self.W)
        out = out if out is not None else torch.empty_like(z)
        sigma_out = sigma_out if sigma_out is not None else torch.empty(self.B, dtype=z.dtype, device=z.device)
        N.call('pnp_csmri_svrg_outer_step', self._h, _p(z), _p(mask_bits), _p(yh), _p(alpha_vec), float(lr), _p(w_out), _p(mu_out),
               _p(out), 1 if denoise else 0, float(sigma_modifier), float(fallback_sigma), _p(xrec), _p(sse), _p(sigma_out), _stream())
        return out, sse, sigma_out


    def svrg_outer_iteration(self, z, w, mu, mask_bits, yh, alpha_vec, selbits, T2, lr, mini_batch_size, xrec, sse_log, log_row0,
                             sigma_out, *, sigma_modifier=1.0, fallback_sigma=0.0):
        assert self.dtype == torch.float32 and self.H == 256 and self.W == 256
        for t in (z, w, mu, xrec):
            assert t.dtype == self.dtype and t.numel() == self.B * self.H * self.W
        assert selbits.dtype == torch.int32 and tuple(selbits.shape) == (T2, self.B, self.W, self.H // 32)
        assert sse_log.dtype == torch.float64 and sse_log.dim() == 2 and sse_log.shape[1] == self.B and sse_log.is_contiguous()
        N.call('pnp_csmri_svrg_outer_iteration', self._h, _p(z), _p(w), _p(mu), _p(mask_bits), _p(yh), _p(alpha_vec), _p(selbits), int(T2),
               float(lr), int(mini_batch_size), float(sigma_modifier), float(fallback_sigma), _p(xrec), _p(sse_log), int(log_row0),
               int(sse_log.shape[0]), _p(sigma_out), _stream())


class DncnnPlan:

    def __init__(self, weights, H, W, batch, winograd=None):
        import numpy as np
        require_gpu()
        n = int(weights['n_layers'])
        self.H, self.W, self.B, self.n_mid = H, W, batch, n - 2
        tr = bool(weights.get('transpose_taps', False))

        def taps(name, shape):
            w = np.asarray(weights[name], dtype=np.float64).reshape(shape + (3, 3))
            return (w.swapaxes(-1, -2) if tr else w).reshape(shape + (9,))

        w_first = np.ascontiguousarray(taps('conv0.weight', (64,)), dtype=np.float32)
        w_last = np.ascontiguousarray(taps(f'conv{n - 1}.weight', (64,)), dtype=np.float32)
        w_mid = np.empty((n - 2, 64, 64, 9), dtype=np.float32)
        b_mid = np.zeros((n - 2, 64), dtype=np.float32)
        for i in range(1, n - 1):
            w = taps(f'conv{i}.weight', (64, 64))
            b = np.asarray(weights[f'conv{i}.bias'], np.float64) if f'conv{i}.bias' in weights else np.zeros(64)
            if f'bn{i}.weight' in weights:
                s = np.asarray(weights[f'bn{i}.weight'], np.float64) / np.sqrt(np.asarray(weights[f'bn{i}.var'], np.float64) + 1e-5)
                w = w * s[:, None, None]
                b = np.asarray(weights[f'bn{i}.bias'], np.float64) + (b - np.asarray(weights[f'bn{i}.mean'], np.float64)) * s
            b_mid[i - 1] = b
            w_mid[i - 1] = w
        h = ctypes.c_void_p()
        N.call('pnp_dncnn_plan_create', ctypes.byref(h), n - 2, w_first.ctypes.data_as(ctypes.c_void_p),
               w_mid.ctypes.data_as(ctypes.c_void_p), b_mid.ctypes.data_as(ctypes.c_void_p),
               w_last.ctypes.data_as(ctypes.c_void_p), H, W, batch)
        self._h = h
        slope = float(weights.get('negative_slope', 0.0))
        if slope != 0.0 or 'conv0.bias' in weights or f'conv{n - 1}.bias' in weights:
            b_first = np.ascontiguousarray(weights.get('conv0.bias', np.zeros(64)), dtype=np.float32)
            b_last = float(np.asarray(weights.get(f'conv{n - 1}.bias', 0.0)).reshape(-1)[0])
            N.call('pnp_dncnn_set_affine', self._h, b_first.ctypes.data_as(ctypes.c_void_p), b_last, slope)
        if winograd is not None:
            N.call('pnp_dncnn_set_winograd', self._h, int(winograd))

    def __del__(self):
        h, self._h = getattr(self, '_h', None), None
        if h:
            try:
                N.lib().pnp_dncnn_plan_destroy(h)
            except Exception:
                pass

    def profile_begin(self, max_calls=4096):
        N.call('pnp_dncnn_profile_begin', self._h, int(max_calls))

    def profile_end(self):
        ms, n = ctypes.c_double(), ctypes.c_long()
        N.call('pnp_dncnn_profile_end', self._h, ctypes.byref(ms), ctypes.byref(n))
        return ms.value, n.value

    def debug_w44_weights(self, layer):
        n = N.lib().pnp_dncnn_debug_w44_floats()
        dst = torch.empty(n, dtype=torch.float32, device='cuda')
        N.call('pnp_dncnn_debug_w44_weights', self._h, int(layer), _p(dst), _stream())
        return dst

    def debug_mid_layer(self, layer, x, out, w44=None, rows=0):
        assert x.dtype == torch.float32 and tuple(x.shape) == (self.B, 64, self.H, self.W) and tuple(out.shape) == tuple(x.shape)
        N.call('pnp_dncnn_debug_mid_layer', self._h, int(layer), _p(x), _p(out), _p(w44), int(rows), _stream())
        return out

    def debug_fused_last(self, x, part, rows=0):
        assert x.dtype == torch.float32 and tuple(x.shape) == (self.B, 64, self.H, self.W)
        assert part.dtype == torch.float32 and part.numel() == self.B * (self.H // 4) * (self.W // 4) * 36
        N.call('pnp_dncnn_debug_fused_last', self._h, _p(x), _p(part), int(rows), _stream())
        return part

    def forward(self, x, out=None):
        assert x.dtype == torch.float32 and tuple(x.shape) == (self.B, self.H, self.W)
        out = out if out is not None else torch.empty_like(x)
        N.call('pnp_dncnn_forward', self._h, _p(x), _p(out), _stream())
        return out

    def denoise(self, z, sigma_net, xrec=None, out=None, sse=None):
        assert tuple(z.shape) == (self.B, self.H, self.W)
        out = out if out is not None else torch.empty_like(z)
        if xrec is not None and sse is None:
            sse = torch.empty(self.B, dtype=torch.float64, device=z.device)
        N.call('pnp_dncnn_denoise', self._h, _p(z), _p(out), _DT[z.dtype], float(sigma_net), _p(xrec), _p(sse), _stream())
        return out, sse


    def mmo_denoise(self, z, xrec=None, out=None, sse=None):
        assert tuple(z.shape) == (self.B, self.H, self.W)
        out = out if out is not None else torch.empty_like(z)
        if xrec is not None and sse is None:
            sse = torch.empty(self.B, dtype=torch.float64, device=z.device)
        N.call('pnp_mmo_denoise', self._h, _p(z), _p(out), _DT[z.dtype], _p(xrec), _p(sse), _stream())
        return out, sse


def sigma_est(z):
    require_gpu()
    B, H, W = z.shape
    out = torch.empty(B, dtype=z.dtype, device=z.device)
    N.call('pnp_sigma_est', _p(z), H, W, B, _DT[z.dtype], _p(out), _stream())
    return out


def prox_tv(z, sigma_in=None, sigma_modifier=1.0, fallback_sigma=0.0, xrec=None, out=None, sse=None, sigma_out=None):
    require_gpu()
    B, H, W = z.shape
    out = out if out is not None else torch.empty_like(z)
    if xrec is not None and sse is None:
        sse = torch.empty(B, dtype=torch.float64, device=z.device)
    sigma_out = sigma_out if sigma_out is not None else torch.empty(B, dtype=z.dtype, device=z.device)
    N.call('pnp_prox_tv', _p(z), _p(out), H, W, B, _DT[z.dtype], _p(sigma_in), float(sigma_modifier),
           float(fallback_sigma), _p(xrec), _p(sse), _p(sigma_out), _stream())
    return out, sse, sigma_out


def sse(z, xrec, out=None):
    require_gpu()
    B = z.shape[0]
    out = out if out is not None else torch.empty(B, dtype=torch.float64, device=z.device)
    N.call('pnp_sse', _p(z), _p(xrec), z.numel() // B, B, _DT[z.dtype], _p(out), _stream())
    return out


def minmax(z):
    require_gpu()
    B = z.shape[0]
    out = torch.empty((B, 2), dtype=z.dtype, device=z.device)
    N.call('pnp_minmax', _p(z), z.numel() // B, B, _DT[z.dtype], _p(out), _stream())
    return out


def axpbypcz(a, x, b=0.0, y=None, c=0.0, w=None, out=None):
    require_gpu()
    out = out if out is not None else torch.empty_like(x)
    N.call('pnp_axpbypcz', float(a), _p(x), float(b), _p(y), float(c), _p(w), _p(out), x.numel(), _DT[x.dtype], _stream())
    return out


_NLM_W0 = {}


def _nlm_w0(side, device):
    key = (side, str(device))
    if key not in _NLM_W0:
        import numpy as np
        off = side // 2
        A = (side - 1.0) / 4.0
        g = np.arange(-off, off + 1)
        gr, gc = np.meshgrid(g, g, indexing='ij')
        w = np.exp(-(gr * gr + gc * gc) / (2 * A * A))
        _NLM_W0[key] = (torch.from_numpy(np.ascontiguousarray(w.ravel())).to(device), float(np.sum(w)))
    return _NLM_W0[key]


def nlm2d(z, sigma_in=None, sigma_modifier=1.0, fixed_h=0.0, patch_size=4, patch_distance=5, xrec=None, out=None, sse=None):
    require_gpu()
    B, H, W = z.shape
    side = patch_size + 1 if patch_size % 2 == 0 else patch_size
    w0, w0_sum = _nlm_w0(side, z.device)
    out = out if out is not None else torch.empty_like(z)
    ws = None
    if xrec is not None:
        sse = sse if sse is not None else torch.empty(B, dtype=torch.float64, device=z.device)
        ws = torch.empty(B * ((H + 15) // 16) * ((W + 15) // 16), dtype=torch.float64, device=z.device)
    N.call('pnp_nlm2d', _p(z), _p(out), H, W, B, _DT[z.dtype], int(patch_size), int(patch_distance), _p(sigma_in),
           float(sigma_modifier), float(fixed_h), _p(w0), w0_sum, _p(xrec), _p(sse), _p(ws), _stream())
    return out, sse


class DeblurPlan:

    def __init__(self, H, W, batch, dtype, Bk, bilinear=None):
        import numpy as np
        require_gpu()
        self.H, self.W, self.N, self.B, self.dtype = H, W, H * W, batch, dtype
        npdt = np.float32 if dtype == torch.float32 else np.float64
        Bk = np.ascontiguousarray(Bk, dtype=npdt)
        h = ctypes.c_void_p()
        vp = lambda a: a.ctypes.data_as(ctypes.c_void_p)
        if bilinear is None:
            self.M = self.N
            N.call('pnp_deblur_plan_create', ctypes.byref(h), H, W, batch, _DT[dtype], vp(Bk), self.M, None, None, None, None, None)
        else:
            g_idx, g_w, a_rowptr, a_col, a_val = bilinear
            self.M = g_idx.shape[0]
            keep = [np.ascontiguousarray(g_idx, np.int32), np.ascontiguousarray(g_w, npdt), np.ascontiguousarray(a_rowptr, np.int32),
                    np.ascontiguousarray(a_col, np.int32), np.ascontiguousarray(a_val, npdt)]
            N.call('pnp_deblur_plan_create', ctypes.byref(h), H, W, batch, _DT[dtype], vp(Bk), self.M, *[vp(k) for k in keep])
        self._h = h

    def __del__(self):
        h, self._h = getattr(self, '_h', None), None
        if h:
            try:
                N.lib().pnp_deblur_plan_destroy(h)
            except Exception:
                pass

    def grad(self, z, Y, sel=None, scale=1.0, out=None, mbd=None):
        assert z.dtype == self.dtype and z.numel() == self.B * self.N and Y.numel() == self.B * self.M
        assert sel is None or mbd is None
        out = out if out is not None else torch.empty_like(z)
        if mbd is not None:
            assert mbd.dtype == torch.int64 and tuple(mbd.shape) == (self.B, 2)
            N.call('pnp_deblur_grad_mb', self._h, _p(z), _p(Y), _p(mbd), float(scale), _p(out), _stream())
        else:
            N.call('pnp_deblur_grad', self._h, _p(z), _p(Y), _p(sel), float(scale), _p(out), _stream())
        return out

    def forward(self, x, out=None):
        out = out if out is not None else torch.empty(self.B * self.M, dtype=self.dtype, device=x.device)
        N.call('pnp_deblur_forward', self._h, _p(x), _p(out), _stream())
        return out


def pr_grad(A, w, y, rows=None, scale=1.0, workspace=None, out=None):
    require_gpu()
    M, Nn = A.shape
    if workspace is None:
        workspace = torch.empty(N.lib().pnp_pr_workspace_elems(M, Nn), dtype=A.dtype, device=A.device)
    out = out if out is not None else torch.empty(Nn, dtype=A.dtype, device=A.device)
    nsel = M if rows is None else rows.numel()
    N.call('pnp_pr_grad', _p(A), _p(w), _p(y), _p(rows), nsel, M, Nn, _DT[A.dtype], float(scale), _p(workspace), _p(out), _stream())
    return out


def pr_grad_batch(A, w, y, rows=None, scale=1.0, workspace=None, out=None):
    require_gpu()
    B, M, Nn = A.shape
    if workspace is None:
        workspace = torch.empty(B * N.lib().pnp_pr_workspace_elems(M, Nn), dtype=A.dtype, device=A.device)
    out = out if out is not None else torch.empty((B, Nn), dtype=A.dtype, device=A.device)
    nsel = M if rows is None else rows.shape[1]
    N.call('pnp_pr_grad_batch', _p(A), _p(w), _p(y), _p(rows), nsel, M, Nn, B, _DT[A.dtype], float(scale), _p(workspace),
           _p(out), _stream())
    return out


def draw_thresholds(M, B, mb, seed, step0, nsteps=1, out=None, step_dev=None, device='cuda'):
    require_gpu()
    out = out if out is not None else torch.empty((nsteps, B, 2), dtype=torch.int64, device=device)
    N.call('pnp_draw_thresholds', int(M), int(B), int(mb), int(seed) & (2 ** 64 - 1), int(step0) & 0xFFFFFFFF, int(nsteps),
           _p(step_dev), _p(out), _stream())
    return out


def indicator_from_thresholds(M, mbd, out=None):
    require_gpu()
    B = mbd.shape[0]
    out = out if out is not None else torch.empty((B, M), dtype=torch.uint8, device=mbd.device)
    N.call('pnp_indicator_from_thresholds', int(M), int(B), _p(mbd), _p(out), _stream())
    return out


def rows_from_thresholds(M, mb, mbd, out=None):
    require_gpu()
    B = mbd.shape[0]
    out = out if out is not None else torch.empty((B, mb), dtype=torch.int32, device=mbd.device)
    N.call('pnp_rows_from_thresholds', int(M), int(B), int(mb), _p(mbd), _p(out), _stream())
    return out


def indicator_from_indices(idx, M, out=None):
    require_gpu()
    assert idx.dtype == torch.int32
    B, n = idx.shape
    out = out if out is not None else torch.empty((B, M), dtype=torch.uint8, device=idx.device)
    N.call('pnp_indicator_from_indices', _p(idx), int(n), int(M), int(B), _p(out), _stream())
    return out


def saga_table_update(z, g, slot, prev, tsum, lr, inv_hist):
    require_gpu()
    for t in (g, slot, prev, tsum):
        assert t.dtype == z.dtype and t.numel() == z.numel()
    N.call('pnp_saga_table_update', _p(z), _p(g), _p(slot), _p(prev), _p(tsum), float(lr), float(inv_hist), z.numel(),
           _DT[z.dtype], _stream())


def pr_spectral_apply(A, v, y, scale=1.0, workspace=None, out=None):
    require_gpu()
    M, Nn = A.shape
    if workspace is None:
        workspace = torch.empty(N.lib().pnp_pr_workspace_elems(M, Nn), dtype=A.dtype, device=A.device)
    out = out if out is not None else torch.empty(Nn, dtype=A.dtype, device=A.device)
    N.call('pnp_pr_spectral_apply', _p(A), _p(v), _p(y), M, Nn, _DT[A.dtype], float(scale), _p(workspace), _p(out), _stream())
    return out


def counter_add(counter, inc=1):
    require_gpu()
    N.call('pnp_counter_add', _p(counter), int(inc), _stream())


def log_append(src, log, step_dev):
    require_gpu()
    N.call('pnp_log_append', _p(src), src.numel(), _p(log), log.shape[0], _p(step_dev), _stream())


def log_append_inc(src, log, counter):
    require_gpu()
    N.call('pnp_log_append_inc', _p(src), src.numel(), _p(log), log.shape[0], _p(counter), _stream())
```

Measured before the change: 5175 inner-iters/s.

## Fuse DnCNN first 1->64 conv into first Winograd F(4x4,3x3) mid layer

Replaces the standalone first-layer conv kernel, which writes a full 64-channel activation tensor, with a small normalization kernel that writes a single-channel image. The first Winograd mid layer then computes the 1->64 conv with bias and ReLU on the fly from that image, using packed FMAs interleaved into its pipeline slots. This removes one large activation write and read per denoiser call. The cost is more work and register/LDS pressure inside the already tightly scheduled mid-layer kernel. It is enabled by default when ReLU and mode 5 are used, with an environment switch to turn it off.

```diff
diff --git a/include/pnp_hip.h b/include/pnp_hip.h
--- a/include/pnp_hip.h
+++ b/include/pnp_hip.h
@@ -109,6 +109,9 @@
 int pnp_dncnn_debug_mid_layer(pnp_dncnn_plan* plan, int layer, const float* in, float* out, const float* w44_override,
                               int w44_rows, void* stream);
 int pnp_dncnn_debug_fused_last(pnp_dncnn_plan* plan, const float* in, float* part, int w44_rows, void* stream);
+int pnp_dncnn_debug_fused_first(pnp_dncnn_plan* plan, const float* x1, float* out, int w44_rows, void* stream);
+int pnp_dncnn_debug_first_layer(pnp_dncnn_plan* plan, const float* x, float* out, void* stream);
+int pnp_dncnn_fuses_first(pnp_dncnn_plan* plan);
 
 int pnp_counter_add(uint32_t* counter, uint32_t inc, void* stream);
 int pnp_log_append(const double* src, int n, double* log, int n_log, const uint32_t* step_dev, void* stream);
diff --git a/pnp_svrg_amd/_native.py b/pnp_svrg_amd/_native.py
--- a/pnp_svrg_amd/_native.py
+++ b/pnp_svrg_amd/_native.py
@@ -59,6 +59,9 @@
     'pnp_dncnn_debug_w44_weights': (_i, [_vp, _i, _vp, _vp]),
     'pnp_dncnn_debug_mid_layer': (_i, [_vp, _i, _vp, _vp, _vp, _i, _vp]),
     'pnp_dncnn_debug_fused_last': (_i, [_vp, _vp, _vp, _i, _vp]),
+    'pnp_dncnn_debug_fused_first': (_i, [_vp, _vp, _vp, _i, _vp]),
+    'pnp_dncnn_debug_first_layer': (_i, [_vp, _vp, _vp, _vp]),
+    'pnp_dncnn_fuses_first': (_i, [_vp]),
     'pnp_draw_thresholds': (_i, [_i, _i, _i, ctypes.c_uint64, ctypes.c_uint32, _i, _vp, _vp, _vp]),
     'pnp_indicator_from_thresholds': (_i, [_i, _i, _vp, _vp, _vp]),
     'pnp_rows_from_thresholds': (_i, [_i, _i, _i, _vp, _vp, _vp]),
diff --git a/pnp_svrg_amd/csrc/dncnn.hip b/pnp_svrg_amd/csrc/dncnn.hip
--- a/pnp_svrg_amd/csrc/dncnn.hip
+++ b/pnp_svrg_amd/csrc/dncnn.hip
@@ -10,6 +10,17 @@
 namespace pnp {
 
 constexpr int C = 64;
+
+template <typename T>
+__device__ __forceinline__ float first_pixel(T u, T lo, T hi, double srange, double sshift, int clamp01) {
+    if (clamp01) {
+        u = u < (T)0 ? (T)0 : (u > (T)1 ? (T)1 : u);
+    } else {
+        u = (u - lo) / (hi - lo);
+        u = u * (T)srange + (T)sshift;
+    }
+    return (float)u;
+}
 
 template <typename T>
 __global__ __launch_bounds__(256) void k_first(const T* __restrict__ z, const T* __restrict__ mm,
@@ -32,16 +43,7 @@
     for (int t = 0; t < 9; ++t) {
         const int yy = y + t / 3 - 1, xx = x + t % 3 - 1;
         float q = 0.f;
-        if (yy >= 0 && yy < H && xx >= 0 && xx < W) {
-            T u = zi[yy * W + xx];
-            if (clamp01) {
-                u = u < (T)0 ? (T)0 : (u > (T)1 ? (T)1 : u);
-            } else {
-                u = (u - lo) / (hi - lo);
-                u = u * (T)srange + (T)sshift;
-            }
-            q = (float)u;
-        }
+        if (yy >= 0 && yy < H && xx >= 0 && xx < W) q = first_pixel<T>(zi[yy * W + xx], lo, hi, srange, sshift, clamp01);
         v[t] = q;
     }
 #pragma unroll 4
@@ -52,6 +54,14 @@
         a += bs[c];
         out[((size_t)b * C + c) * H * W + p] = a > 0.f ? a : slope * a + 0.f;
     }
+}
+
+__global__ __launch_bounds__(256) void k_norm1(const float* __restrict__ z, const float* __restrict__ mm, float* __restrict__ x1,
+                                               int HW, double srange, double sshift) {
+    const int b = blockIdx.y, p = blockIdx.x * 256 + threadIdx.x;
+    if (p >= HW) return;
+    const float lo = mm ? mm[2 * b] : 0.f, hi = mm ? mm[2 * b + 1] : 1.f;
+    x1[(size_t)b * HW + p] = first_pixel<float>(z[(size_t)b * HW + p], lo, hi, srange, sshift, 0);
 }
 
 constexpr int LT_R = 16, LT_C = 64, LT_CK = 4, LT_PR = LT_R + 2, LT_PC = LT_C + 8;
@@ -215,10 +225,10 @@
 using namespace pnp;
 
 static const ConvMode kModes[] = {
-    {0, direct_supports, direct_layer_bytes, direct_pack, direct_layer, direct_debug_clock, false},
-    {1, direct_supports, wino23_layer_bytes, wino23_pack, wino23_layer, wino23_debug_clock, false},
-    {5, wino44_supports, wino44_layer_bytes, wino44_pack, wino44_layer, wino44_debug_clock, true},
-    {6, wino44b_supports, wino44b_layer_bytes, wino44b_pack, wino44b_layer, wino44b_debug_clock, false},
+    {0, direct_supports, direct_layer_bytes, direct_pack, direct_layer, direct_debug_clock, false, false},
+    {1, direct_supports, wino23_layer_bytes, wino23_pack, wino23_layer, wino23_debug_clock, false, false},
+    {5, wino44_supports, wino44_layer_bytes, wino44_pack, wino44_layer, wino44_debug_clock, true, true},
+    {6, wino44b_supports, wino44b_layer_bytes, wino44b_pack, wino44b_layer, wino44b_debug_clock, false, false},
 };
 constexpr int NMODES = sizeof(kModes) / sizeof(kModes[0]);
 
@@ -246,7 +256,10 @@
     float* b_first;
     float b_last, slope;
     bool edge_fusion;
+    bool first_fusion;
     float* part;
+    float *x1, *first_tab;
+    std::vector<float> w_first_h, b_first_h;
     float *act0, *act1, *zeros;
     double* mm;
     double* sse_part;
@@ -260,7 +273,7 @@
 static void plan_free(pnp_dncnn_plan* p) {
     for (void* q : p->wconv) (void)hipFree(q);
     for (void* q : {(void*)p->bias, (void*)p->w_first, (void*)p->w_last, (void*)p->act0, (void*)p->act1, (void*)p->zeros,
-                    (void*)p->mm, (void*)p->sse_part, (void*)p->b_first, (void*)p->part})
+                    (void*)p->mm, (void*)p->sse_part, (void*)p->b_first, (void*)p->part, (void*)p->x1, (void*)p->first_tab})
         (void)hipFree(q);
     for (hipEvent_t e : p->ev) (void)hipEventDestroy(e);
     delete p;
@@ -286,6 +299,10 @@
     (void)resolve_conv_mode(ev ? atoi(ev) : 5, H, W, false, &p->conv);
     const char* ef = getenv("PNP_DNCNN_EDGE_FUSION");
     p->edge_fusion = !(ef && atoi(ef) == 0);
+    const char* ff = getenv("PNP_DNCNN_FIRST_FUSION");
+    p->first_fusion = p->edge_fusion && !(ff && atoi(ff) == 0);
+    p->w_first_h.assign(w_first, w_first + C * 9);
+    p->b_first_h.assign(C, 0.f);
     const size_t act_bytes = (size_t)batch * C * H * W * sizeof(float);
     hipError_t e = hipSuccess;
     auto alloc = [&](auto** dst, size_t bytes, const void* src = nullptr) {
@@ -309,7 +326,13 @@
     if (e == hipSuccess) e = hipMemset(p->zeros, 0, 256);
     alloc(&p->mm, (size_t)batch * 2 * sizeof(double));
     alloc(&p->sse_part, (size_t)batch * (H * W / 256) * sizeof(double));
-    if (wino44_supports(H, W)) alloc(&p->part, wino44_part_floats(H, W, batch) * sizeof(float));
+    if (wino44_supports(H, W)) {
+        alloc(&p->part, wino44_part_floats(H, W, batch) * sizeof(float));
+        alloc(&p->x1, (size_t)batch * H * W * sizeof(float));
+        std::vector<float> tab(wino44_first_tab_floats());
+        wino44_pack_first(p->w_first_h.data(), p->b_first_h.data(), tab.data());
+        alloc(&p->first_tab, tab.size() * sizeof(float), tab.data());
+    }
     if (e != hipSuccess) {
         set_error(std::string("pnp_dncnn_plan_create: ") + hipGetErrorString(e));
         plan_free(p);
@@ -322,6 +345,10 @@
 extern "C" int pnp_dncnn_plan_destroy(pnp_dncnn_plan* p) {
     if (p) plan_free(p);
     return PNP_OK;
+}
+
+static bool plan_fuses_first(const pnp_dncnn_plan* p) {
+    return p->first_fusion && p->conv->fuses_first && p->slope == 0.f && p->x1 != nullptr && p->n_mid >= 2;
 }
 
 namespace {
@@ -338,16 +365,21 @@
         sshift = (1.0 - srange) / 2.0;
     }
     dim3 pg(HW / 256, B);
-    k_first<T><<<pg, 256, 0, s>>>(z_in, mm, p->w_first, p->b_first, p->act0, H, W, srange, sshift, mmo ? 1 : 0, p->slope);
+    const bool fuse_last = p->edge_fusion && p->conv->fuses_last && p->slope == 0.f && !mmo && std::is_same<T, float>::value &&
+                           p->part != nullptr;
+    const bool fuse_first = plan_fuses_first(p) && !mmo && std::is_same<T, float>::value;
+    if constexpr (std::is_same<T, float>::value) {
+        if (fuse_first) k_norm1<<<pg, 256, 0, s>>>(z_in, mm, p->x1, HW, srange, sshift);
+    }
+    if (!fuse_first) k_first<T><<<pg, 256, 0, s>>>(z_in, mm, p->w_first, p->b_first, p->act0, H, W, srange, sshift, mmo ? 1 : 0, p->slope);
     PNP_CHECK_LAUNCH();
     float *src = p->act0, *dst = p->act1;
-    const bool fuse_last = p->edge_fusion && p->conv->fuses_last && p->slope == 0.f && !mmo && std::is_same<T, float>::value &&
-                           p->part != nullptr;
     const bool prof = p->profile && p->ev_used + 2 <= p->ev.size();
     if (prof) PNP_CHECK_HIP(hipEventRecord(p->ev[p->ev_used], s));
     for (int l = 0; l < p->n_mid; ++l) {
         ConvLayerArgs a = conv_args(p, l, src, dst, s);
         if (fuse_last && l == p->n_mid - 1) { a.wlast = p->w_last; a.part = p->part; }
+        if (fuse_first && l == 0) { a.x1 = p->x1; a.first_tab = p->first_tab; }
         const int rc = p->conv->layer(a);
         if (rc != PNP_OK) return rc;
         std::swap(src, dst);
@@ -405,11 +437,38 @@
     return p->conv->layer(a);
 }
 
+extern "C" int pnp_dncnn_fuses_first(pnp_dncnn_plan* p) { return p && plan_fuses_first(p) ? 1 : 0; }
+
+extern "C" int pnp_dncnn_debug_first_layer(pnp_dncnn_plan* p, const float* x, float* out, void* stream) {
+    PNP_CHECK_ARG(p && x && out, "bad argument");
+    k_first<float><<<dim3(p->H * p->W / 256, p->batch), 256, 0, (hipStream_t)stream>>>(x, nullptr, p->w_first, p->b_first, out, p->H,
+                                                                                         p->W, 1.0, 0.0, 0, p->slope);
+    PNP_CHECK_LAUNCH();
+    return PNP_OK;
+}
+
+extern "C" int pnp_dncnn_debug_fused_first(pnp_dncnn_plan* p, const float* x1, float* out, int w44_rows, void* stream) {
+    PNP_CHECK_ARG(p && x1 && out && w44_rows >= 0 && w44_rows <= 2, "bad argument");
+    PNP_CHECK_ARG(p->conv->fuses_first && p->first_tab != nullptr, "the fused first layer needs the F(4x4,3x3) kernel (mode 5)");
+    ConvLayerArgs a = conv_args(p, 0, nullptr, out, (hipStream_t)stream);
+    a.force_rows = w44_rows;
+    a.x1 = x1;
+    a.first_tab = p->first_tab;
+    return p->conv->layer(a);
+}
+
 extern "C" int pnp_dncnn_set_affine(pnp_dncnn_plan* p, const float* b_first, float b_last, float negative_slope) {
     PNP_CHECK_ARG(p != nullptr, "null plan");
     PNP_CHECK_ARG(negative_slope >= 0.f && negative_slope < 1.f, "negative_slope must be in [0, 1)");
     if (b_first) PNP_CHECK_HIP(hipMemcpy(p->b_first, b_first, C * sizeof(float), hipMemcpyHostToDevice));
     else PNP_CHECK_HIP(hipMemset(p->b_first, 0, C * sizeof(float)));
+    if (b_first) p->b_first_h.assign(b_first, b_first + C);
+    else p->b_first_h.assign(C, 0.f);
+    if (p->first_tab) {
+        std::vector<float> tab(wino44_first_tab_floats());
+        wino44_pack_first(p->w_first_h.data(), p->b_first_h.data(), tab.data());
+        PNP_CHECK_HIP(hipMemcpy(p->first_tab, tab.data(), tab.size() * sizeof(float), hipMemcpyHostToDevice));
+    }
     p->b_last = b_last;
     p->slope = negative_slope;
     return PNP_OK;
@@ -449,7 +508,14 @@
 extern "C" int pnp_dncnn_debug_clock(pnp_dncnn_plan* p, int reps, double* cycles, double* ref_ticks, void* stream) {
     PNP_CHECK_ARG(p && cycles && ref_ticks && reps >= 1, "bad argument");
     std::vector<double> c, r;
-    const int rc = p->conv->debug_clock(conv_args(p, 0, p->act0, p->act1, (hipStream_t)stream), reps, c, r);
+    ConvLayerArgs a = conv_args(p, 0, p->act0, p->act1, (hipStream_t)stream);
+    const char* wf = getenv("PNP_W44_FIRST");
+    if (wf && atoi(wf) != 0) {
+        PNP_CHECK_ARG(p->conv->fuses_first && p->x1 != nullptr && p->slope == 0.f, "PNP_W44_FIRST needs the F(4x4,3x3) kernel (mode 5) and ReLU");
+        a.x1 = p->x1;
+        a.first_tab = p->first_tab;
+    }
+    const int rc = p->conv->debug_clock(a, reps, c, r);
     if (rc != PNP_OK) return rc;
     std::sort(c.begin(), c.end());
     std::sort(r.begin(), r.end());
diff --git a/pnp_svrg_amd/csrc/dncnn_conv.h b/pnp_svrg_amd/csrc/dncnn_conv.h
--- a/pnp_svrg_amd/csrc/dncnn_conv.h
+++ b/pnp_svrg_amd/csrc/dncnn_conv.h
@@ -17,6 +17,8 @@
     const float* w44_override = nullptr;
     const float* wlast = nullptr;
     float* part = nullptr;
+    const float* x1 = nullptr;
+    const float* first_tab = nullptr;
 };
 
 struct ConvMode {
@@ -27,11 +29,13 @@
     int (*layer)(const ConvLayerArgs& a);
     int (*debug_clock)(const ConvLayerArgs& a, int reps, std::vector<double>& cycles, std::vector<double>& ticks);
     bool fuses_last;
+    bool fuses_first;
 };
 
 inline int check_plain_conv(const ConvLayerArgs& a) {
     PNP_CHECK_ARG(a.w44_override == nullptr, "w44_override needs the F(4x4,3x3) kernel (mode 5)");
     PNP_CHECK_ARG(a.part == nullptr, "the fused last layer needs the F(4x4,3x3) kernel (mode 5) and ReLU");
+    PNP_CHECK_ARG(a.x1 == nullptr, "the fused first layer needs the F(4x4,3x3) kernel (mode 5) and ReLU");
     return PNP_OK;
 }
 
diff --git a/pnp_svrg_amd/csrc/dncnn_wino44.hip b/pnp_svrg_amd/csrc/dncnn_wino44.hip
--- a/pnp_svrg_amd/csrc/dncnn_wino44.hip
+++ b/pnp_svrg_amd/csrc/dncnn_wino44.hip
@@ -74,6 +74,17 @@
     f32x2 t[6][3];
     f32x2 v[6];
 };
+typedef __attribute__((address_space(4))) const f32x2 const_f2;
+struct First {
+    f32x2 x[2][8];
+    f32x2 a[12];
+    f32x2 w[10];
+    f32x4 o[2][3];
+    const lds_f* xsrc[2];
+    lds_f* dst;
+    float hi[2][3];
+    const_f2* wtab;
+};
 template <int NG_> struct Ctx {
     static constexpr int NG = NG_;
     using G = Geo<NG_>;
@@ -87,6 +98,7 @@
     const lds_f* vsrc1[2];
     const __attribute__((address_space(1))) char* ucur;
     unsigned ulane;
+    First F;
     __device__ __forceinline__ f32x4 uload_next() {
         const f32x4 u = *(const __attribute__((address_space(1))) f32x4*)(ucur + ulane);
         ucur += 1024;
@@ -170,7 +182,95 @@
     if constexpr (GR < CT::NG) mfma<CT::G::in_agpr(GR, XI)>(c.acc[GR][XI], u, b[GR].y);
 }
 
-template <int K, int P, int VAR, typename CT, typename DMA> __device__ __forceinline__ void step(CT& c, DMA&& dma) {
+constexpr int XC = 80;
+constexpr int XBUF = 1024;
+template <int NG, bool FIRST> constexpr int first_lds_floats() { return FIRST ? 2 * XBUF : 0; }
+constexpr int FIRST_TAB_FLOATS = (C / 2) * 10 * 2;
+
+template <int SEL, bool ZERO> __device__ __forceinline__ void first_tap(f32x2& acc, f32x2 x, f32x2 w) {
+    if constexpr (ZERO) {
+        if constexpr (SEL == 0) asm("v_pk_fma_f32 %0, %1, %2, 0 op_sel_hi:[0,1,1]" : "=v"(acc) : "v"(x), "s"(w));
+        else asm("v_pk_fma_f32 %0, %1, %2, 0 op_sel:[1,0,0]" : "=v"(acc) : "v"(x), "s"(w));
+    } else {
+        if constexpr (SEL == 0) asm("v_pk_fma_f32 %0, %1, %2, %0 op_sel_hi:[0,1,1]" : "+v"(acc) : "v"(x), "s"(w));
+        else asm("v_pk_fma_f32 %0, %1, %2, %0 op_sel:[1,0,0]" : "+v"(acc) : "v"(x), "s"(w));
+    }
+}
+template <int XS, int R, int PART, typename CT> __device__ __forceinline__ void first_read(CT& c) {
+    const lds_f* row = c.F.xsrc[XS] + R * XC;
+    f32x2 (&x)[8] = c.F.x[R & 1];
+    if constexpr (PART == 0) x[0] = *(const lds_f2*)row;
+    else if constexpr (PART == 4) x[7] = *(const lds_f2*)(row + 14);
+    else {
+        const f32x4 m = *(const lds_f4*)(row + 4 * PART - 2);
+        x[2 * PART - 1] = f32x2{m.x, m.y};
+        x[2 * PART] = f32x2{m.z, m.w};
+    }
+}
+template <int KC2, typename CT> __device__ __forceinline__ void first_weights(CT& c) {
+#pragma unroll
+    for (int i = 0; i < 10; ++i) c.F.w[i] = c.F.wtab[KC2 * 40 + i];
+}
+template <int XS, int DY, typename CT> __device__ __forceinline__ void first_block(CT& c) {
+    f32x2 (&x)[8] = c.F.x[DY & 1];
+#pragma unroll
+    for (int dx = 0; dx < 3; ++dx)
+#pragma unroll
+        for (int i = 0; i < 12; ++i) {
+            const int n = i + 1 + dx;
+            if (DY == 0 && dx == 0) { if (n & 1) first_tap<1, true>(c.F.a[i], x[n >> 1], c.F.w[0]); else first_tap<0, true>(c.F.a[i], x[n >> 1], c.F.w[0]); }
+            else { if (n & 1) first_tap<1, false>(c.F.a[i], x[n >> 1], c.F.w[3 * DY + dx]); else first_tap<0, false>(c.F.a[i], x[n >> 1], c.F.w[3 * DY + dx]); }
+        }
+    if constexpr (DY == 2) {
+#pragma unroll
+        for (int i = 0; i < 12; ++i) {
+            const f32x2 v = c.F.a[i] + c.F.w[9];
+            c.F.o[0][i >> 2][i & 3] = __builtin_amdgcn_fmed3f(v.x, 0.f, c.F.hi[XS][i >> 2]);
+            c.F.o[1][i >> 2][i & 3] = __builtin_amdgcn_fmed3f(v.y, 0.f, c.F.hi[XS][i >> 2]);
+        }
+    }
+}
+template <int DPAR, int N, typename CT> __device__ __forceinline__ void first_write(CT& c) {
+    *(lds_f4*)(c.F.dst + DPAR * CT::G::DBUF + (N / 3) * CT::G::PLANE + 4 * (N % 3)) = c.F.o[N / 3][N % 3];
+}
+template <int K, int P, int N, typename CT> __device__ __forceinline__ void first_slot(CT& c) {
+    constexpr int XS = K + 2 < NCH ? 0 : 1, KC2 = (K + 2) % NCH, DPAR = K & 1;
+    if constexpr (P == 11) {
+        if constexpr (N == 0) { first_weights<KC2>(c); first_read<XS, 0, 0>(c); first_read<XS, 0, 1>(c); }
+        else first_read<XS, 0, N + 1>(c);
+    } else if constexpr (P == 12) first_read<XS, 1, N>(c);
+    else if constexpr (P == 13) {
+        if constexpr (N == 0) first_block<XS, 0>(c);
+        else if constexpr (N == 1) first_read<XS, 1, 4>(c);
+        else first_read<XS, 2, N - 2>(c);
+    } else if constexpr (P == 14) {
+        if constexpr (N == 0) first_block<XS, 1>(c);
+        else first_read<XS, 2, N + 1>(c);
+    } else if constexpr (P == 15) {
+        if constexpr (N == 0) first_block<XS, 2>(c);
+        else first_write<DPAR, N - 1>(c);
+    } else if constexpr (P == 16) {
+        if constexpr (N > 0) first_write<DPAR, N + 2>(c);
+    }
+}
+template <int R, typename CT, int... I> __device__ __forceinline__ void first_row_now(CT& c, std::integer_sequence<int, I...>) {
+    (first_read<0, R, I>(c), ...);
+}
+template <int DPAR, typename CT, int... I> __device__ __forceinline__ void first_writes_now(CT& c, std::integer_sequence<int, I...>) {
+    (first_write<DPAR, I>(c), ...);
+}
+template <int KC2, int DPAR, typename CT> __device__ __forceinline__ void first_chunk_now(CT& c) {
+    first_weights<KC2>(c);
+    first_row_now<0>(c, std::make_integer_sequence<int, 5>{});
+    first_row_now<1>(c, std::make_integer_sequence<int, 5>{});
+    first_block<0, 0>(c);
+    first_row_now<2>(c, std::make_integer_sequence<int, 5>{});
+    first_block<0, 1>(c);
+    first_block<0, 2>(c);
+    first_writes_now<DPAR>(c, std::make_integer_sequence<int, 6>{});
+}
+
+template <int K, int P, int VAR, bool FIRST, typename CT, typename DMA> __device__ __forceinline__ void step(CT& c, DMA&& dma) {
     constexpr int X0 = 2 * P, X1 = 2 * P + 1, SQ = K * 18 + P;
     constexpr int VPAR = K & 1, DPAR = (K + 1) & 1, NG = CT::NG;
     const f32x4 u = c.ur[SQ % URING];
@@ -185,9 +285,11 @@
     PNP_SLOT();
     mfma_j1<X0, 0>(c, u.y, b0);                      PNP_SLOT();
     if constexpr (VAR != 10 && VAR != 15) slice_valu<P>(c);
+    if constexpr (FIRST) first_slot<K, P, 0>(c);
     PNP_SLOT();
     mfma_j1<X0, 1>(c, u.y, b0);                      PNP_SLOT();
     if constexpr (VAR != 14 && VAR != 15) slice_lds<DPAR, P, 0>(c);
+    if constexpr (FIRST) first_slot<K, P, 1>(c);
     PNP_SLOT();
 #pragma unroll
     for (int g = 0; g < NG; ++g) b1[g] = c.b[1][g];
@@ -198,37 +300,41 @@
     if constexpr (X1 + 1 < 36 && VAR != 13 && VAR != 15) b_load<VPAR, X1 + 1, 1>(c);
     PNP_SLOT();
     mfma_j1<X1, 0>(c, u.w, b1);                      PNP_SLOT();
-    if constexpr (P < CT::G::PPW && VAR != 11 && VAR != 15) dma(P);
+    if constexpr (FIRST) { if constexpr (K == 0 && P == 0) dma(0); }
+    else if constexpr (P < CT::G::PPW && VAR != 11 && VAR != 15) dma(P);
     if constexpr (VAR != 14 && VAR != 15) slice_lds<DPAR, P, 1>(c);
+    if constexpr (FIRST) first_slot<K, P, 2>(c);
     PNP_SLOT();
     mfma_j1<X1, 1>(c, u.w, b1);                      PNP_SLOT();
     if constexpr (VAR != 14 && VAR != 15) slice_lds<DPAR, P, 2>(c);
+    if constexpr (FIRST) first_slot<K, P, 3>(c);
     if constexpr (VAR != 12 && VAR != 15 && SQ + URING < NCH * 18) c.ur[SQ % URING] = c.uload_next();
     PNP_SLOT();
 }
-template <int K, int VAR, typename CT, typename DMA, int... P> __device__ __forceinline__ void chunk_steps(CT& c, DMA&& dma, std::integer_sequence<int, P...>) {
-    (step<K, P, VAR>(c, dma), ...);
+template <int K, int VAR, bool FIRST, typename CT, typename DMA, int... P> __device__ __forceinline__ void chunk_steps(CT& c, DMA&& dma, std::integer_sequence<int, P...>) {
+    (step<K, P, VAR, FIRST>(c, dma), ...);
 }
 template <int K> constexpr int reloads_from(int p0) {
     int n = 0;
     for (int p = p0; p < 18; ++p) n += (K * 18 + p + URING < NCH * 18) ? 1 : 0;
     return n;
 }
-template <int K, bool STAMP, int VAR, typename CT, typename DMA> __device__ __forceinline__ void chunk(CT& c, DMA&& dma, unsigned long long& t_wait) {
+template <int K, bool STAMP, int VAR, bool FIRST, typename CT, typename DMA> __device__ __forceinline__ void chunk(CT& c, DMA&& dma, unsigned long long& t_wait) {
     patch_load<(K + 1) & 1, 0, 0>(c);
     patch_load<(K + 1) & 1, 0, 1>(c);
     b_load<K & 1, 0, 0>(c);
     b_load<K & 1, 0, 1>(c);
     PNP_SLOT();
-    chunk_steps<K, VAR>(c, dma, std::make_integer_sequence<int, 18>{});
+    chunk_steps<K, VAR, FIRST>(c, dma, std::make_integer_sequence<int, 18>{});
     unsigned long long ta = 0;
     if (STAMP) ta = __builtin_amdgcn_s_memtime();
-    asm volatile("s_waitcnt vmcnt(%0)" :: "n"(reloads_from<K>(CT::G::PPW)) : "memory");
+    if constexpr (!FIRST) asm volatile("s_waitcnt vmcnt(%0)" :: "n"(reloads_from<K>(CT::G::PPW)) : "memory");
+    else if constexpr (K == 0) asm volatile("s_waitcnt vmcnt(%0)" :: "n"(reloads_from<K>(1)) : "memory");
     __syncthreads();
     if (STAMP) t_wait += __builtin_amdgcn_s_memtime() - ta;
 }
-template <bool STAMP, int VAR, typename CT, typename MK, int... K> __device__ __forceinline__ void all_chunks(CT& c, MK&& mk, unsigned long long& t_wait, std::integer_sequence<int, K...>) {
-    (chunk<K, STAMP, VAR>(c, mk(std::integral_constant<int, K>{}), t_wait), ...);
+template <bool STAMP, int VAR, bool FIRST, typename CT, typename MK, int... K> __device__ __forceinline__ void all_chunks(CT& c, MK&& mk, unsigned long long& t_wait, std::integer_sequence<int, K...>) {
+    (chunk<K, STAMP, VAR, FIRST>(c, mk(std::integral_constant<int, K>{}), t_wait), ...);
 }
 
 template <int VPL> __device__ __forceinline__ void transform0(const float* dsrc, float* vdst) {
@@ -251,16 +357,16 @@
 constexpr int FL_BLK = 16 * FL_PATCH;
 template <int NG, bool FL> constexpr int fl_lds_floats() { return FL ? C * 9 + NG * 4 * FL_BLK : 0; }
 
-template <bool LEAKY, int NG = 2, bool STAMP = false, int VAR = 0, bool FL = false>
-__global__ __launch_bounds__(256, 1) void k_mid_wino44(const float* __restrict__ in, float* __restrict__ out,
-                                                       const float4* __restrict__ upack, const float* __restrict__ bias,
-                                                       int H, int W, int ntiles, float slope,
-                                                       unsigned long long* __restrict__ stamps = nullptr, int tile0 = 0,
-                                                       const float* __restrict__ wlast = nullptr, float* __restrict__ part = nullptr) {
+template <bool LEAKY, int NG, bool STAMP, int VAR, bool FL, bool FIRST>
+__device__ __forceinline__ void mid_wino44_body(const float* __restrict__ in, float* __restrict__ out,
+                                                const float4* __restrict__ upack, const float* __restrict__ bias,
+                                                int H, int W, int ntiles, float slope, unsigned long long* __restrict__ stamps, int tile0,
+                                                const float* __restrict__ wlast, float* __restrict__ part, const float* __restrict__ ftab) {
     using G = Geo<NG>;
     constexpr int TR = G::TR, PR = G::PR, PLANE = G::PLANE, DBUF = G::DBUF, PPW = G::PPW, VPL = G::VPL, VBUF = G::VBUF;
-    static_assert(!(FL && LEAKY), "the fused last layer is built for the ReLU net");
-    __shared__ __attribute__((aligned(16))) float lds[G::LDS_FLOATS + fl_lds_floats<NG, FL>()];
+    static_assert(!(FL && LEAKY) && !(FIRST && LEAKY), "the fused edge layers are built for the ReLU net");
+    constexpr int XOFF = G::LDS_FLOATS + fl_lds_floats<NG, FL>();
+    __shared__ __attribute__((aligned(16))) float lds[XOFF + first_lds_floats<NG, FIRST>()];
     const int tid = threadIdx.x, lane = tid & 63, wv = __builtin_amdgcn_readfirstlane(tid >> 6);
     const int tiles_x = W / TC, units_per_img = tiles_x * (H / 8);
     auto region = [&](int u, int& b, int& ty0, int& tx0) {
@@ -335,7 +441,51 @@
     float* const flx = flw + C * 9;
     if constexpr (FL)
         for (int i = tid; i < C * 9; i += 256) flw[i] = wlast[i];
-    {
+    constexpr int NL = PR * 6;
+    const int fl = lane < NL ? lane : 0, fry = fl / 6, fg = fl - 6 * fry;
+    const int xr = tid / 20, xc4 = 4 * (tid - 20 * xr);
+    lds_f* const xl = ldsp + XOFF + fry * XC + 12 * fg + 2;
+    int xb = 0;
+    auto first_hi = [&](int t, float (&hi)[3]) {
+        int b, ty0, tx0;
+        region(t, b, ty0, tx0);
+        const int y = ty0 - 1 + fry;
+        const bool row = y >= 0 && y < H;
+        hi[0] = row && !(fg == 0 && tx0 == 0) ? __builtin_inff() : 0.f;
+        hi[1] = row ? __builtin_inff() : 0.f;
+        hi[2] = row && !(fg == 5 && tx0 + TC == W) ? __builtin_inff() : 0.f;
+    };
+    struct XDma { size_t base; unsigned voff; };
+    auto x_dma = [&](int t) {
+        XDma xd;
+        int b, ty0, tx0;
+        region(t, b, ty0, tx0);
+        const int y = ty0 - 2 + xr, x = tx0 - 8 + xc4;
+        xd.base = (size_t)in + 4 * (((size_t)b * H + ty0 - 2) * (size_t)W + tx0 - 8);
+        xd.voff = t < ntiles && xr < PR + 2 && y >= 0 && y < H && x >= 0 && x < W ? 4u * (unsigned)(xr * W + xc4) : 0x80000000u;
+        return xd;
+    };
+    auto x_piece = [&](const XDma& xd, int buf) {
+        i32x4 rs;
+        rs.x = (int)(unsigned)xd.base; rs.y = (int)(unsigned)(xd.base >> 32) & 0xFFFF; rs.z = (int)0x80000000u; rs.w = 0x00020000;
+        dma_piece_asm(xd.voff, rs, lds0 + 4u * (unsigned)(XOFF + buf * XBUF + wv * 256));
+    };
+    if constexpr (FIRST) {
+        c.F.wtab = (const_f2*)(size_t)ftab + wv * 10;
+        c.F.dst = ldsp + 2 * wv * PLANE + fry * PC + 12 * fg;
+        c.F.xsrc[0] = xl;
+        first_hi(tile < limit ? tile : ntiles, c.F.hi[0]);
+        x_piece(x_dma(tile < limit ? tile : ntiles), 0);
+#pragma unroll
+        for (int i = 0; i < URING; ++i) c.ur[i] = c.uload_next();
+        asm volatile("s_waitcnt vmcnt(0)" ::: "memory");
+        __syncthreads();
+        first_chunk_now<0, 0>(c);
+        first_chunk_now<1, 1>(c);
+        __syncthreads();
+        transform0<VPL>(dbuf + d_off, vbuf + v_off);
+        __syncthreads();
+    } else {
         const TileDma td0 = tile_dma(tile < limit ? tile : ntiles);
 #pragma unroll
         for (int i = 0; i < PPW; ++i) dma_piece(td0, chunk_rsrc(td0, 0), 0, i);
@@ -357,13 +507,23 @@
         region(tile, b, ty0, tx0);
         const int ntile = tile + tw_.step < limit ? tile + tw_.step : ntiles;
 
+        if constexpr (FIRST) {
+            asm volatile("" : "+s"(c.F.wtab));
+            first_hi(tile, c.F.hi[0]); first_hi(ntile, c.F.hi[1]);
+            c.F.xsrc[0] = xl + xb * XBUF; c.F.xsrc[1] = xl + (xb ^ 1) * XBUF;
+            const XDma xd = x_dma(ntile);
+            all_chunks<STAMP, VAR, true>(c, [&](auto) { return [&](int) { x_piece(xd, xb ^ 1); }; }, t_wait,
+                                         std::make_integer_sequence<int, NCH>{});
+            xb ^= 1;
+        } else {
         const TileDma cur = tile_dma(tile), nxt = tile_dma(ntile);
-        all_chunks<STAMP, VAR>(c, [&](auto kc) {
+        all_chunks<STAMP, VAR, false>(c, [&](auto kc) {
             constexpr int K = decltype(kc)::value;
             const TileDma& td = K + 2 < NCH ? cur : nxt;
             const i32x4 rs = chunk_rsrc(td, (K + 2) % NCH);
             return [&, rs](int piece) { dma_piece(td, rs, K & 1, piece); };
         }, t_wait, std::make_integer_sequence<int, NCH>{});
+        }
 
         unsigned long long te = 0;
         if (STAMP) te = __builtin_amdgcn_s_memtime();
@@ -489,6 +649,22 @@
         stamps[4 * blockIdx.x + 2] = t_wait;
         stamps[4 * blockIdx.x + 3] = t_epi;
     }
+}
+
+template <bool LEAKY, int NG = 2, bool STAMP = false, int VAR = 0, bool FL = false>
+__global__ __launch_bounds__(256, 1) void k_mid_wino44(const float* __restrict__ in, float* __restrict__ out,
+                                                       const float4* __restrict__ upack, const float* __restrict__ bias,
+                                                       int H, int W, int ntiles, float slope,
+                                                       unsigned long long* __restrict__ stamps = nullptr, int tile0 = 0,
+                                                       const float* __restrict__ wlast = nullptr, float* __restrict__ part = nullptr) {
+    mid_wino44_body<LEAKY, NG, STAMP, VAR, FL, false>(in, out, upack, bias, H, W, ntiles, slope, stamps, tile0, wlast, part, nullptr);
+}
+template <int NG = 2, bool STAMP = false>
+__global__ __launch_bounds__(256, 1) void k_mid_wino44_first(const float* __restrict__ x1, float* __restrict__ out,
+                                                             const float4* __restrict__ upack, const float* __restrict__ bias,
+                                                             int H, int W, int ntiles, const float* __restrict__ ftab,
+                                                             unsigned long long* __restrict__ stamps = nullptr, int tile0 = 0) {
+    mid_wino44_body<false, NG, STAMP, 0, false, true>(x1, out, upack, bias, H, W, ntiles, 0.f, stamps, tile0, nullptr, nullptr, ftab);
 }
 
 }
@@ -519,9 +695,21 @@
                     }
 }
 
+size_t wino44_first_tab_floats() { return w44::FIRST_TAB_FLOATS; }
+
+void wino44_pack_first(const float* w_first, const float* b_first, float* tab) {
+    for (int p = 0; p < w44::C / 2; ++p)
+        for (int j = 0; j < 2; ++j) {
+            for (int t = 0; t < 9; ++t) tab[(p * 10 + t) * 2 + j] = w_first[(2 * p + j) * 9 + t];
+            tab[(p * 10 + 9) * 2 + j] = b_first[2 * p + j];
+        }
+}
+
 int wino44_layer(const ConvLayerArgs& a) {
     PNP_CHECK_ARG(a.part == nullptr || (a.slope == 0.f && a.wlast != nullptr), "the fused last layer needs ReLU and w_last");
-    const float *in = a.in, *bias = a.bias, *wlast = a.wlast;
+    PNP_CHECK_ARG(a.x1 == nullptr || (a.slope == 0.f && a.first_tab != nullptr && a.part == nullptr),
+                  "the fused first layer needs ReLU and its weight table, and is not combined with the fused last layer");
+    const float *in = a.in, *bias = a.bias, *wlast = a.wlast, *x1 = a.x1, *ftab = a.first_tab;
     float *out = a.out, *part = a.part;
     const int H = a.H, W = a.W, num_cu = a.num_cu, force = a.force_rows, batch = a.batch;
     const float slope = a.slope;
@@ -532,14 +720,16 @@
     const float4* up = (const float4*)(a.w44_override ? a.w44_override : (const float*)a.w + a.layer * wino44_layer_bytes() / sizeof(float));
     if (full > 0) {
         const int grid = full < num_cu ? full : num_cu;
-        if (part) w44::k_mid_wino44<false, 2, false, 0, true><<<grid, 256, 0, s>>>(in, out, up, bias, H, W, full, 0.f, nullptr, 0, wlast, part);
+        if (x1) w44::k_mid_wino44_first<2><<<grid, 256, 0, s>>>(x1, out, up, bias, H, W, full, ftab, nullptr, 0);
+        else if (part) w44::k_mid_wino44<false, 2, false, 0, true><<<grid, 256, 0, s>>>(in, out, up, bias, H, W, full, 0.f, nullptr, 0, wlast, part);
         else if (slope != 0.f) w44::k_mid_wino44<true, 2><<<grid, 256, 0, s>>>(in, out, up, bias, H, W, full, slope, nullptr, 0);
         else w44::k_mid_wino44<false, 2><<<grid, 256, 0, s>>>(in, out, up, bias, H, W, full, 0.f, nullptr, 0);
         PNP_CHECK_LAUNCH();
     }
     if (full < units) {
         const int n1 = 2 * (units - full), grid = n1 < num_cu ? n1 : num_cu;
-        if (part) w44::k_mid_wino44<false, 1, false, 0, true><<<grid, 256, 0, s>>>(in, out, up, bias, H, W, n1, 0.f, nullptr, full, wlast, part);
+        if (x1) w44::k_mid_wino44_first<1><<<grid, 256, 0, s>>>(x1, out, up, bias, H, W, n1, ftab, nullptr, full);
+        else if (part) w44::k_mid_wino44<false, 1, false, 0, true><<<grid, 256, 0, s>>>(in, out, up, bias, H, W, n1, 0.f, nullptr, full, wlast, part);
         else if (slope != 0.f) w44::k_mid_wino44<true, 1><<<grid, 256, 0, s>>>(in, out, up, bias, H, W, n1, slope, nullptr, full);
         else w44::k_mid_wino44<false, 1><<<grid, 256, 0, s>>>(in, out, up, bias, H, W, n1, 0.f, nullptr, full);
         PNP_CHECK_LAUNCH();
@@ -557,10 +747,13 @@
     const float* upack_layer = (const float*)a.w + a.layer * wino44_layer_bytes() / sizeof(float);
     std::vector<unsigned long long> h;
     const int rc = read_stamps(s, grid, 4, [&](unsigned long long* stamps_dev) {
-        for (int i = 0; i < reps - 1; ++i)
-            w44::k_mid_wino44<false, 2><<<grid, 256, 0, s>>>(in, out, (const float4*)upack_layer, bias, H, W, ntiles, 0.f);
+        for (int i = 0; i < reps - 1; ++i) {
+            if (a.x1) w44::k_mid_wino44_first<2><<<grid, 256, 0, s>>>(a.x1, out, (const float4*)upack_layer, bias, H, W, ntiles, a.first_tab);
+            else w44::k_mid_wino44<false, 2><<<grid, 256, 0, s>>>(in, out, (const float4*)upack_layer, bias, H, W, ntiles, 0.f);
+        }
         const int var = getenv("PNP_W44_VAR") ? atoi(getenv("PNP_W44_VAR")) : 0;
-        if (var == 0) w44::k_mid_wino44<false, 2, true><<<grid, 256, 0, s>>>(in, out, (const float4*)upack_layer, bias, H, W, ntiles, 0.f, stamps_dev);
+        if (a.x1) w44::k_mid_wino44_first<2, true><<<grid, 256, 0, s>>>(a.x1, out, (const float4*)upack_layer, bias, H, W, ntiles, a.first_tab, stamps_dev);
+        else if (var == 0) w44::k_mid_wino44<false, 2, true><<<grid, 256, 0, s>>>(in, out, (const float4*)upack_layer, bias, H, W, ntiles, 0.f, stamps_dev);
 #ifdef PNP_W44_ABLATIONS
 #define PNP_W44_ABL(V) else if (var == V) w44::k_mid_wino44<false, 2, true, V><<<grid, 256, 0, s>>>(in, out, (const float4*)upack_layer, bias, H, W, ntiles, 0.f, stamps_dev);
         PNP_W44_ABL(10) PNP_W44_ABL(11) PNP_W44_ABL(12) PNP_W44_ABL(13) PNP_W44_ABL(14) PNP_W44_ABL(15)
diff --git a/pnp_svrg_amd/csrc/wino44.h b/pnp_svrg_amd/csrc/wino44.h
--- a/pnp_svrg_amd/csrc/wino44.h
+++ b/pnp_svrg_amd/csrc/wino44.h
@@ -6,6 +6,8 @@
 size_t wino44_layer_bytes();
 void wino44_pack(const float* w_mid, int n_mid, void* out);
 int wino44_layer(const ConvLayerArgs& a);
+size_t wino44_first_tab_floats();
+void wino44_pack_first(const float* w_first, const float* b_first, float* tab);
 inline size_t wino44_part_floats(int H, int W, int batch) { return (size_t)batch * (H / 4) * (W / 4) * 36; }
 int wino44_debug_clock(const ConvLayerArgs& a, int reps, std::vector<double>& cycles, std::vector<double>& ticks);
 }
diff --git a/pnp_svrg_amd/ops.py b/pnp_svrg_amd/ops.py
--- a/pnp_svrg_amd/ops.py
+++ b/pnp_svrg_amd/ops.py
@@ -211,6 +211,22 @@
         N.call('pnp_dncnn_debug_fused_last', self._h, _p(x), _p(part), int(rows), _stream())
         return part
 
+    def debug_fused_first(self, x1, out, rows=0):
+        assert x1.dtype == torch.float32 and tuple(x1.shape) == (self.B, self.H, self.W)
+        assert out.dtype == torch.float32 and tuple(out.shape) == (self.B, 64, self.H, self.W)
+        N.call('pnp_dncnn_debug_fused_first', self._h, _p(x1), _p(out), int(rows), _stream())
+        return out
+
+    def debug_first_layer(self, x, out):
+        assert x.dtype == torch.float32 and tuple(x.shape) == (self.B, self.H, self.W)
+        assert out.dtype == torch.float32 and tuple(out.shape) == (self.B, 64, self.H, self.W)
+        N.call('pnp_dncnn_debug_first_layer', self._h, _p(x), _p(out), _stream())
+        return out
+
+    @property
+    def fuses_first(self):
+        return bool(N.lib().pnp_dncnn_fuses_first(self._h))
+
     def forward(self, x, out=None):
         assert x.dtype == torch.float32 and tuple(x.shape) == (self.B, self.H, self.W)
         out = out if out is not None else torch.empty_like(x)
```

New measurement: 5198 inner-iters/s, median of 6. No clear change (+0.5%).
